# autonomousvision/unimatch

Hardware: AMD Instinct MI355X
Metric: image_pairs_per_sec (higher is better)
Workload: dtype f16x2

## Files before the change

### include/unimatch_hip.h

```cpp
#ifndef UNIMATCH_HIP_H
#define UNIMATCH_HIP_H

#include <stddef.h>
#include <stdint.h>

#ifdef __cplusplus
extern "C" {
#endif

#define UM_VERSION 220

#define UM_MODE_EXACT 0
#define UM_MODE_FAST 1

#define UM_ERR_BAD_ARG (-1)
#define UM_ERR_BAD_GEOMETRY (-2)
#define UM_ERR_WORKSPACE (-3)
#define UM_ERR_UNSUPPORTED (-4)
#define UM_ERR_COLLECTIVE (-5)

int um_version(void);
const char* um_last_error_string(void);

#define UM_RANGE_PLANES 1u
// ... 60 lines not shown
                             const float* gamma, const float* beta, const float* residual, float eps, int wshift, float* out,
                             int streams, int h, int w, int channels, int ldq, int ldkv, long q_plane_stride,
                             long kv_plane_stride, int win_h, int win_w, int shift_h, int shift_w, int kv_rotate, int mode,
                             void* stream);

size_t um_window_attn_ksplit_workspace_bytes(int streams, int h, int w, int win_h, int win_w);
int um_window_attn_plan(int streams, int h, int w, int win_h, int win_w, int* full_tiles, int* split_tiles, int* parts);
int um_window_attn_qproj_merge_fwd(const float* x, const void* wq_planes, const void* k_planes, const void* v_planes,
                                   const void* wm_planes, const float* gamma, const float* beta, const float* residual, float eps,
                                   int wshift, float* out, int streams, int h, int w, int channels, int ldkv,
                                   long kv_plane_stride, int win_h, int win_w, int shift_h, int shift_w, int kv_rotate, int mode,
                                   void* workspace, size_t workspace_bytes, void* stream);

#define UM_EPI_PLANES 0
#define UM_EPI_LN 1
#define UM_EPI_GELU_PLANES 2
size_t um_planes_bytes(long rows, int cols, int mode);
int um_weight_planes(const float* w, void* planes, int n, int k, int wshift, int mode, void* stream);
int um_linear_fwd(const float* a0, const float* a1, const void* a_planes, const void* w_planes,
                  int m, int n, int k, int wshift, int epilogue, void* out,
                  const float* gamma, const float* beta, const float* residual, float eps,
                  int mode, void* stream);

int um_linear_bias_fwd(const float* a0, const void* a_planes, const void* w_planes, const float* bias, int m, int n, int k,
                       int wshift, float out_mul, float bias_mul, void* out_planes, float* out_f32, int mode, void* stream);

int um_ffn_fwd(const float* x, const float* y, const void* w1_planes, const void* w2_planes, int m, int hidden,
               int wshift, const float* gamma, const float* beta, float eps, float* out, int mode, void* stream);
size_t um_ffn_split_workspace_bytes(int m, int hidden);
int um_ffn_ws_fwd(const float* x, const float* y, const void* w1_planes, const void* w2_planes, int m, int hidden,
                  int wshift, const float* gamma, const float* beta, float eps, float* out, int mode, void* workspace,
                  size_t workspace_bytes, void* stream);

int um_kv4_fwd(const float* x, const void* wc_planes, int m, int wshift, void* out_planes, int mode, void* stream);
int um_ffn_kv_fwd(const float* x, const float* y, const void* w1_planes, const void* w2_planes, int m, int hidden, int wshift,
                  const float* gamma, const float* beta, float eps, float* out, const void* wc_planes, void* kv_planes, int mode,
                  void* workspace, size_t workspace_bytes, void* stream);

int um_conv2d_fwd(const void* a_planes, const void* w_planes, const float* bias, float* out, float* stats_out, int batch,
                  int hi, int wi, int cin, int cout, int kh, int kw, int stride, int pad_h, int pad_w, int relu, int wshift,
                  int mode, void* stream);
int um_conv2d_ex(const void* a_planes, int a_ld, int a_coff, long a_rows, const void* w_planes, const float* bias, float* out,
                 int out_ld, int out_coff, void* out_planes, int outp_ld, int outp_coff, long outp_rows, float* stats_out,
                 int batch, int hi, int wi, int cin, int cout, int kh, int kw, int stride, int pad_h, int pad_w, int act,
                 int wshift, int mode, void* stream);
int um_conv2d_gru_fwd(int gate, const void* a_planes, int a_ld, int a_coff, long a_rows, const void* w_planes, const float* bias,
                      float* hidden, const float* z, int z_ld, float* z_out, int z_out_ld, void* out_planes, int outp_ld,
                      int outp_coff, long outp_rows, int batch, int hi, int wi, int cin, int channels, int kh, int kw, int pad_h,
                      int pad_w, int wshift, int mode, void* stream);
int um_conv2d_gru_add_fwd(int gate, const void* a_planes, int a_ld, int a_coff, long a_rows, const void* w_planes, const float* bias,
                          const float* addend, int addend_ld, float* hidden, const float* z, int z_ld, float* z_out, int z_out_ld,
                          void* out_planes, int outp_ld, int outp_coff, long outp_rows, int batch, int hi, int wi, int cin,
                          int channels, int kh, int kw, int pad_h, int pad_w, int wshift, int mode, void* stream);
int um_conv_stats_parts(int hi, int wi, int cout, int kh, int kw, int stride, int pad_h, int pad_w);
size_t um_conv_stats_bytes(int batch, int parts, int channels);

size_t um_stem_planes_bytes(int batch, int h, int w);
size_t um_conv7_planes_bytes(int batch, int h, int w, int stride);
int um_conv7_fwd(const float* image, int channels, int normalize, const float* mean3, const float* std3, void* image_planes,
                 const void* w_planes, const float* bias, float* out, int out_ld, int out_coff, void* out_planes, int outp_ld,
                 int outp_coff, long outp_rows, float* stats_out, int batch, int h, int w, int cout, int stride, int act,
                 int wshift, void* stream);
int um_stem_conv_fwd(const float* image, int normalize, const float* mean3, const float* std3, void* image_planes,
                     const void* w_planes, float* out, float* stats_out, int batch, int h, int w, int cout, int wshift,
                     void* stream);

size_t um_nhwc_norm_workspace_bytes(int batch, int pixels, int channels);
int um_nhwc_instance_norm(const float* x, const float* shortcut, const void* shortcut_planes, void* planes_out, float* f32_out,
                          int batch, int pixels, int channels, float eps, int normalize, int relu, const float* conv_stats,
                          int conv_stats_parts, void* workspace, size_t workspace_bytes, int mode, void* stream);

size_t um_nhwc_norm_sc_workspace_bytes(int batch, int pixels, int channels);
int um_nhwc_instance_norm_sc(const float* x, const float* shortcut, const void* shortcut_planes, void* planes_out, float* f32_out,
                             int batch, int pixels, int channels, float eps, int normalize, int relu, const float* conv_stats,
                             int conv_stats_parts, void* workspace, size_t workspace_bytes, int mode, void* stream,
                             const float* sc_conv_stats, int sc_conv_stats_parts);

int um_nhwc_stats_finalize(const float* conv_stats, int conv_stats_parts, float* stats_out, int batch, int pixels, int channels,
                           float eps, void* stream);
int um_conv2d_norm_supported(int hi, int wi, int cin, int cout, int kh, int kw, int stride, int pad_h, int pad_w, int mode);
int um_conv2d_norm_fwd(const float* x, const float* norm_stats, int norm_relu, const void* w_planes, const float* bias, float* out,
                       float* stats_out, int batch, int hi, int wi, int cin, int cout, int kh, int kw, int stride, int pad_h,
                       int pad_w, int relu, int wshift, int mode, void* stream);

int um_conv2d_entry_supported(int hi, int wi, int cin, int cout, int kh, int kw, int stride, int pad_h, int pad_w, int mode);
int um_conv2d_entry_fwd(const float* u, const float* ustats, const void* s_planes, const void* w_planes, const void* w2_planes,
                        const float* bias2, float* out_t, float* out_d, float* stats_t, float* stats_d, int batch, int hi, int wi,
                        int cin, int cout, int kh, int kw, int stride, int pad_h, int pad_w, int wshift, int mode, void* stream);

int um_nhwc_gate(int mode, const float* src, int src_ld, const float* zr, float* hbuf, void* planes_out, int ld, int coff,
                 long plane_rows, long rows, int channels, void* stream);

int um_nchw_to_nhwc(const float* x, void* planes_out, float* f32_out, int batch, int channels, int pixels, int mode,
                    void* stream);

size_t um_global_corr_workspace_bytes(int batch, int tokens, int channels, int mode);
int um_global_corr_softmax_flow(const float* f0, const float* f1, float* flow,
                                int batch, int h, int w, int channels, int bidir,
                                int mode, void* workspace, size_t workspace_bytes, void* stream);

int um_global_corr_softmax_stereo(const float* f0, const float* f1, float* disp,
                                  int batch, int h, int w, int channels,
                                  int mode, void* workspace, size_t workspace_bytes, void* stream);

int um_prop_global_attn(const float* q, const float* k, const float* value, float* out,
                        int batch, int h, int w, int channels, int value_channels,
                        int mode, void* workspace, size_t workspace_bytes, void* stream);
float um_global_corr_plane_scale(int channels);
int um_prop_global_attn_planes(const void* q_planes, const void* k_planes, const float* value, float* out, int batch, int h,
                               int w, int channels, int value_channels, int mode, void* workspace, size_t workspace_bytes,
                               void* stream);


int um_local_corr_softmax(const float* f0, const float* f1, float* out,
                          int batch, int h, int w, int channels, int radius, int one_d, void* stream);

int um_local_corr_with_flow(const float* f0, const float* f1, const float* flow, float* cost,
                            int batch, int h, int w, int channels, int radius, void* stream);
int um_local_corr_with_flow_dilated(const float* f0, const float* f1, const float* flow, float* cost,
                                    int batch, int h, int w, int channels, int radius, int dilation, void* stream);
int um_local_corr_with_flow_planes(const float* f0, const float* f1, const float* flow, void* planes_out, int ld, long plane_rows,
                                   int batch, int h, int w, int channels, int radius, void* stream);

// ... 102 lines not shown
```

### unimatch_amd/_abi.py

```python
import ctypes
import os

_HERE = os.path.dirname(os.path.abspath(__file__))
LIB_PATH = os.environ.get('UM_LIB') or os.path.join(_HERE, 'libunimatch_hip.so')

MODE_EXACT = 0
MODE_FAST = 1

CENSUS = {'wattn_tile': 0, 'wattn_ksplit': 1, 'ffn_tile': 2, 'ffn_hsplit': 3, 'gsv4': 4, 'gsv3': 5, 'k4_mfma': 6, 'k4_valu': 7,
          'k3_mfma': 8, 'k3_valu': 9, 'conv_patch': 10, 'conv_rows': 11, 'conv_generic': 12, 'wattn_w8': 13, 'conv_patch_norm': 14}

_c_int, _c_size_t, _c_void_p = ctypes.c_int, ctypes.c_size_t, ctypes.c_void_p

SIGNATURES = {
    'um_version': (_c_int, []),
    'um_last_error_string': (ctypes.c_char_p, []),
    'um_range_flags': (_c_int, [ctypes.POINTER(ctypes.c_uint), _c_int]),
    'um_timing_enable': (_c_int, [_c_int]),
    'um_timing_collect': (_c_int, [_c_int, ctypes.POINTER(ctypes.c_double), ctypes.POINTER(_c_int)]),
    'um_window_attn_workspace_bytes': (_c_size_t, [_c_int] * 4),
    'um_window_attn_fwd': (_c_int, [_c_void_p] * 4 + [_c_int] * 9 + [_c_void_p, _c_size_t, _c_void_p]),
    'um_window_attn_planes_fwd': (_c_int, [_c_void_p] * 4 + [_c_int] * 6 + [ctypes.c_long] * 2 + [_c_int] * 6 + [_c_void_p]),
    'um_window_attn_merge_fwd': (_c_int, [_c_void_p] * 7 + [ctypes.c_float, _c_int, _c_void_p] + [_c_int] * 6 + [ctypes.c_long] * 2 +
                                 [_c_int] * 6 + [_c_void_p]),
    'um_window_attn_qproj_merge_fwd': (_c_int, [_c_void_p] * 8 + [ctypes.c_float, _c_int, _c_void_p] + [_c_int] * 5 + [ctypes.c_long] +
                                       [_c_int] * 6 + [_c_void_p, _c_size_t, _c_void_p]),
    'um_window_attn_ksplit_workspace_bytes': (_c_size_t, [_c_int] * 5),
    'um_window_attn_plan': (_c_int, [_c_int] * 5 + [ctypes.POINTER(_c_int)] * 3),
    'um_planes_bytes': (_c_size_t, [ctypes.c_long, _c_int, _c_int]),
    'um_weight_planes': (_c_int, [_c_void_p] * 2 + [_c_int] * 4 + [_c_void_p]),
    'um_linear_fwd': (_c_int, [_c_void_p] * 4 + [_c_int] * 5 + [_c_void_p] * 4 + [ctypes.c_float, _c_int, _c_void_p]),
    'um_linear_bias_fwd': (_c_int, [_c_void_p] * 4 + [_c_int] * 4 + [ctypes.c_float] * 2 + [_c_void_p] * 2 + [_c_int, _c_void_p]),
    'um_ffn_fwd': (_c_int, [_c_void_p] * 4 + [_c_int] * 3 + [_c_void_p] * 2 + [ctypes.c_float, _c_void_p, _c_int, _c_void_p]),
    'um_ffn_ws_fwd': (_c_int, [_c_void_p] * 4 + [_c_int] * 3 + [_c_void_p] * 2 + [ctypes.c_float, _c_void_p, _c_int, _c_void_p, _c_size_t,
                                _c_void_p]),
    'um_ffn_split_workspace_bytes': (_c_size_t, [_c_int] * 2),
    'um_ffn_kv_fwd': (_c_int, [_c_void_p] * 4 + [_c_int] * 3 + [_c_void_p] * 2 + [ctypes.c_float, _c_void_p, _c_void_p, _c_void_p, _c_int, _c_void_p,
                                _c_size_t, _c_void_p]),
    'um_kv4_fwd': (_c_int, [_c_void_p, _c_void_p, _c_int, _c_int, _c_void_p, _c_int, _c_void_p]),
    'um_conv2d_fwd': (_c_int, [_c_void_p] * 5 + [_c_int] * 13 + [_c_void_p]),
    'um_conv2d_ex': (_c_int, [_c_void_p, _c_int, _c_int, ctypes.c_long, _c_void_p, _c_void_p, _c_void_p, _c_int, _c_int, _c_void_p,
                              _c_int, _c_int, ctypes.c_long, _c_void_p] + [_c_int] * 13 + [_c_void_p]),
    'um_nhwc_gate': (_c_int, [_c_int, _c_void_p, _c_int, _c_void_p, _c_void_p, _c_void_p, _c_int, _c_int, ctypes.c_long, ctypes.c_long,
                              _c_int, _c_void_p]),
    'um_local_corr_with_flow_planes': (_c_int, [_c_void_p] * 4 + [_c_int, ctypes.c_long] + [_c_int] * 5 + [_c_void_p]),
    'um_conv2d_gru_fwd': (_c_int, [_c_int, _c_void_p, _c_int, _c_int, ctypes.c_long, _c_void_p, _c_void_p, _c_void_p, _c_void_p, _c_int,
                                   _c_void_p, _c_int, _c_void_p, _c_int, _c_int, ctypes.c_long] + [_c_int] * 11 + [_c_void_p]),
    'um_conv2d_gru_add_fwd': (_c_int, [_c_int, _c_void_p, _c_int, _c_int, ctypes.c_long, _c_void_p, _c_void_p, _c_void_p, _c_int, _c_void_p, _c_void_p,
                                        _c_int, _c_void_p, _c_int, _c_void_p, _c_int, _c_int, ctypes.c_long] + [_c_int] * 11 + [_c_void_p]),
    'um_conv2d_norm_supported': (_c_int, [_c_int] * 10),
    'um_conv2d_norm_fwd': (_c_int, [_c_void_p, _c_void_p, _c_int] + [_c_void_p] * 4 + [_c_int] * 13 + [_c_void_p]),
    'um_conv2d_entry_supported': (_c_int, [_c_int] * 10),
    'um_conv2d_entry_fwd': (_c_int, [_c_void_p] * 10 + [_c_int] * 12 + [_c_void_p]),
    'um_nhwc_norm_sc_workspace_bytes': (_c_size_t, [_c_int] * 3),
    'um_nhwc_instance_norm_sc': (_c_int, [_c_void_p] * 5 + [_c_int] * 3 + [ctypes.c_float, _c_int, _c_int, _c_void_p, _c_int, _c_void_p,
                                          _c_size_t, _c_int, _c_void_p, _c_void_p, _c_int]),
    'um_nhwc_stats_finalize': (_c_int, [_c_void_p, _c_int, _c_void_p] + [_c_int] * 3 + [ctypes.c_float, _c_void_p]),
    'um_conv_stats_bytes': (_c_size_t, [_c_int] * 3),
    'um_conv_stats_parts': (_c_int, [_c_int] * 8),
    'um_stem_planes_bytes': (_c_size_t, [_c_int] * 3),
    'um_conv7_planes_bytes': (_c_size_t, [_c_int] * 4),
    'um_conv7_fwd': (_c_int, [_c_void_p, _c_int, _c_int] + [_c_void_p] * 6 + [_c_int, _c_int, _c_void_p, _c_int, _c_int, ctypes.c_long,
                              _c_void_p] + [_c_int] * 7 + [_c_void_p]),
    'um_stem_conv_fwd': (_c_int, [_c_void_p, _c_int] + [_c_void_p] * 6 + [_c_int] * 5 + [_c_void_p]),
    'um_nhwc_norm_workspace_bytes': (_c_size_t, [_c_int] * 3),
    'um_nhwc_instance_norm': (_c_int, [_c_void_p] * 5 + [_c_int] * 3 + [ctypes.c_float, _c_int, _c_int, _c_void_p, _c_int, _c_void_p,
                                       _c_size_t, _c_int, _c_void_p]),
    'um_nchw_to_nhwc': (_c_int, [_c_void_p] * 3 + [_c_int] * 4 + [_c_void_p]),
    'um_flow_warp': (_c_int, [_c_void_p] * 3 + [_c_int] * 4 + [_c_void_p]),
    'um_fwd_bwd_occlusion': (_c_int, [_c_void_p] * 4 + [_c_int] * 3 + [ctypes.c_float] * 2 + [_c_void_p]),
    'um_flow_to_rgb_workspace_bytes': (_c_size_t, [_c_int] * 3),
    'um_flow_to_rgb': (_c_int, [_c_void_p] * 2 + [_c_int] * 3 + [_c_void_p, _c_size_t, _c_void_p]),
    'um_flow_metrics_workspace_bytes': (_c_size_t, [_c_int] * 3),
    'um_flow_metrics': (_c_int, [_c_void_p] * 5 + [_c_int] * 7 + [_c_void_p, _c_size_t, _c_void_p]),
    'um_disp_metrics_workspace_bytes': (_c_size_t, [_c_int] * 3),
    'um_disp_metrics': (_c_int, [_c_void_p] * 3 + [_c_int] * 7 + [ctypes.c_float, _c_void_p, _c_size_t, _c_void_p]),
    'um_depth_metrics_workspace_bytes': (_c_size_t, [_c_int] * 3),
    'um_depth_metrics': (_c_int, [_c_void_p] * 4 + [_c_int] * 7 + [ctypes.c_float] * 2 + [_c_void_p, _c_size_t, _c_void_p]),
    'um_image_prepare': (_c_int, [_c_void_p, _c_int, _c_void_p] + [_c_int] * 4 + [ctypes.POINTER(ctypes.c_float)] * 2 + [_c_int] * 5 +
                         [_c_void_p]),
    'um_pred_restore': (_c_int, [_c_void_p] * 2 + [_c_int] * 11 + [_c_void_p]),
    'um_convex_upsample': (_c_int, [_c_void_p] * 3 + [_c_int] * 7 + [_c_void_p]),
    'um_flow_upsample2x': (_c_int, [_c_void_p] * 2 + [_c_int] * 4 + [ctypes.c_float, _c_void_p]),
    'um_depth_cam_pack': (_c_int, [_c_void_p] * 3 + [_c_int, ctypes.c_float, _c_int, _c_void_p]),
    'um_rigid_flow': (_c_int, [_c_void_p] * 3 + [_c_int] * 3 + [_c_void_p]),
    'um_instance_norm_fwd': (_c_int, [_c_void_p] * 3 + [ctypes.c_long, _c_int, ctypes.c_float, _c_int, _c_void_p]),
    'um_global_corr_workspace_bytes': (_c_size_t, [_c_int] * 4),
    'um_global_corr_softmax_flow': (_c_int, [_c_void_p] * 3 + [_c_int] * 6 + [_c_void_p, _c_size_t, _c_void_p]),
    'um_global_corr_softmax_stereo': (_c_int, [_c_void_p] * 3 + [_c_int] * 5 + [_c_void_p, _c_size_t, _c_void_p]),
    'um_prop_global_attn': (_c_int, [_c_void_p] * 4 + [_c_int] * 6 + [_c_void_p, _c_size_t, _c_void_p]),
    'um_global_corr_plane_scale': (ctypes.c_float, [_c_int]),
    'um_prop_global_attn_planes': (_c_int, [_c_void_p] * 4 + [_c_int] * 6 + [_c_void_p, _c_size_t, _c_void_p]),
    'um_local_corr_softmax': (_c_int, [_c_void_p] * 3 + [_c_int] * 6 + [_c_void_p]),
    'um_local_corr_with_flow': (_c_int, [_c_void_p] * 4 + [_c_int] * 5 + [_c_void_p]),
    'um_local_corr_with_flow_dilated': (_c_int, [_c_void_p] * 4 + [_c_int] * 6 + [_c_void_p]),
    'um_local_corr_feat_planes_bytes': (ctypes.c_size_t, [_c_int] * 4),
    'um_local_corr_feat_planes': (_c_int, [_c_void_p] * 3 + [_c_int] * 4 + [_c_void_p]),
    'um_local_corr_with_flow_feat_supported': (_c_int, [_c_int] * 4),
    'um_local_corr_softmax_mfma': (_c_int, [_c_void_p] * 3 + [_c_int] * 5 + [_c_void_p, ctypes.c_size_t, _c_void_p]),
    'um_local_corr_with_flow_feat': (_c_int, [_c_void_p] * 6 + [_c_int, ctypes.c_long] + [_c_int] * 6 + [_c_void_p, _c_void_p]),
    'um_prop_local_attn': (_c_int, [_c_void_p] * 4 + [_c_int] * 6 + [_c_void_p]),
    'um_depth_corr_softmax': (_c_int, [_c_void_p] * 5 + [_c_int] * 6 + [_c_void_p]),
    'um_census_enable': (_c_int, [_c_int]),
    'um_census_count': (ctypes.c_long, [_c_int]),
    'um_window_attn_tile_census': (_c_int, [_c_int, ctypes.POINTER(ctypes.c_ulonglong)]),
    'um_probe_mfma_flops': (ctypes.c_double, [_c_int]),
    'um_probe_mfma': (_c_int, [_c_void_p, _c_int, _c_void_p]),
    'um_probe_copy': (_c_int, [_c_void_p, _c_void_p, _c_size_t, _c_void_p]),
    'um_probe_chase': (_c_int, [_c_void_p, _c_void_p, _c_int, _c_void_p]),
    'um_swin_attn_fwd': (_c_int, [_c_void_p] * 4 + [_c_int] * 9 + [_c_void_p, _c_size_t, _c_void_p]),
    'um_attn1d_fwd': (_c_int, [_c_void_p] * 4 + [_c_int] * 7 + [_c_void_p, _c_size_t, _c_void_p]),
    'um_local_corr_softmax_1d': (_c_int, [_c_void_p] * 3 + [_c_int] * 5 + [_c_void_p]),
    **{f'um_workspace_bytes_{op}': (_c_size_t, [_c_int] * 5) for op in (
        'swin_attn_fwd', 'attn1d_fwd', 'global_corr_softmax_flow', 'global_corr_softmax_stereo', 'prop_global_attn',
        'local_corr_softmax', 'local_corr_softmax_1d', 'local_corr_with_flow', 'prop_local_attn', 'depth_corr_softmax',
        'allgather_preds')},
    'um_comm_unique_id': (_c_int, [_c_void_p]),
# ... 100 lines not shown
```

### unimatch_amd/csrc/conv.hip

```cpp
#include <cstdlib>
#include <cstring>
#ifndef UM_CONV_2P
#define UM_CONV_2P 0
#endif
#include "common.h"
#include "planes.h"

struct ConvArgs {
    const unsigned short* ap;
    long a_plane_stride;
    unsigned row_stride;
    unsigned zero_row;
    const unsigned short* wp;
    long w_plane_stride;
    const float* bias;
    float* out;
    unsigned short* outp;
    long outp_plane_stride;
    int out_ld, out_coff, outp_ld, outp_coff;
    int act;
    int gate, gate_c, gate_zld;
    float* gate_h;
    const float* gate_z;
    float* gate_hout;
    int gate_hout_ld;
    float* stats;
    const float* addend;
    int addend_ld;
    int B, Hi, Wi, Cin, Ho, Wo, Cout;
    int KH, KW, stride, pad_h, pad_w;
    int M;
    float out_scale;
    int xcd;
    const float* xf;
    const float* nstats;
    int norm_relu;
};

__device__ __forceinline__ void conv_dma16(const void* base, unsigned byte_off, const unsigned char* lds_dst) {
    const unsigned dst = __builtin_amdgcn_readfirstlane(
        (unsigned)(unsigned long)(const __attribute__((address_space(3))) unsigned char*)lds_dst);
    unsigned keep;
    asm volatile("s_mov_b32 %0, m0\n\ts_mov_b32 m0, %3\n\ts_nop 0\n\tglobal_load_lds_dwordx4 %1, %2\n\ts_mov_b32 m0, %0"
                 : "=&s"(keep)
                 : "v"(byte_off), "s"(base), "s"(dst)
                 : "memory");
}

template <int V>
struct IntC {
    static constexpr int value = V;
};

template <typename T, int NS, int NT, int NT0, int NTP, int WSTRIDE>
__device__ __forceinline__ void conv_epilogue_pass(const ConvArgs& a, f32x16 (&acc)[NT], unsigned char* lds, unsigned char* scratch,
                                                   int bt, int rloc0, int nvalid, int part0, bool dense_parts, int n0, int tid,
                                                   int wave, int lane, int half) {
    const int P = a.Ho * a.Wo;
    constexpr int ROWB = 32 * NTP * 4;
    const int nb = n0 + 32 * NT0;
    unsigned char* stg = lds + wave * WSTRIDE;
    const int tl = lane & 31;
    constexpr int CPR = 8 * NTP;
    constexpr int ITER = 32 * CPR / 64;
    constexpr int BATCH = ITER < 4 ? ITER : 4, NBATCH = ITER / BATCH, NSIDE = NT == 4 ? 2 : 1;
    static_assert(ITER % BATCH == 0, "batches cover the iterations");
    const long rowbase = (long)bt * P + rloc0;
    const int nrows = nvalid;
    const int gate = a.gate;
    float* hbase = gate ? a.gate_h + rowbase * a.gate_c : nullptr;
    const float* zbase = gate == 2 ? a.gate_z + rowbase * a.gate_zld : nullptr;
    const float* abase = a.addend ? a.addend + rowbase * a.addend_ld : nullptr;
    float* hobase = gate == 2 ? a.gate_hout + rowbase * a.gate_hout_ld : nullptr;
    f32x4 ad[NSIDE][BATCH], gz[NSIDE][BATCH], gh[NSIDE][BATCH];
    auto preload = [&](int b, int slot) {
        if (!abase && !gate) return;
#pragma unroll
        for (int j = 0; j < BATCH; ++j) {
            const int idx = (b * BATCH + j) * 64 + lane;
            const int r = idx / CPR, c = idx - r * CPR;
            const int col = nb + 4 * c;
            if (r < nrows && col < a.Cout) {
                if (abase) ad[slot][j] = *reinterpret_cast<const f32x4*>(abase + (unsigned)(r * a.addend_ld + col));
                if (gate == 1 && col >= a.gate_c) gh[slot][j] = *reinterpret_cast<const f32x4*>(hbase + (unsigned)(r * a.gate_c + col - a.gate_c));
                if (gate == 2) {
                    gz[slot][j] = *reinterpret_cast<const f32x4*>(zbase + (unsigned)(r * a.gate_zld + col));
                    gh[slot][j] = *reinterpret_cast<const f32x4*>(hbase + (unsigned)(r * a.gate_c + col));
                }
            }
        }
    };
    preload(0, 0);
    auto to_lds = [&](auto act_tag, auto bias_tag) {
        constexpr int ACT = decltype(act_tag)::value;
        constexpr bool BIAS = decltype(bias_tag)::value != 0;
#pragma unroll
        for (int nt = 0; nt < NTP; ++nt)
#pragma unroll
            for (int g = 0; g < 4; ++g) {
                const int n = nb + 32 * nt + 8 * g + 4 * half;
                f32x4 v;
#pragma unroll
                for (int i = 0; i < 4; ++i) v[i] = acc[NT0 + nt][4 * g + i] * a.out_scale;
                if (BIAS) v = v + *reinterpret_cast<const f32x4*>(a.bias + min(n, a.Cout - 4));
#pragma unroll
                for (int i = 0; i < 4; ++i) {
                    if (ACT == 1) v[i] = fmaxf(v[i], 0.f);
                    else if (ACT == 2) v[i] = 1.0f / (1.0f + __expf(-v[i]));
                    else if (ACT == 3) v[i] = tanhf(v[i]);
                }
                const int c = 8 * nt + 2 * g + half;
                *reinterpret_cast<f32x4*>(stg + tl * ROWB + ((c ^ (tl & 7)) << 4)) = v;
            }
    };
    auto to_lds_b = [&](auto act_tag) {
        if (a.bias) to_lds(act_tag, IntC<1>{});
        else to_lds(act_tag, IntC<0>{});
    };
    switch (a.addend ? 0 : a.act) {
        case 0: to_lds_b(IntC<0>{}); break;
        case 1: to_lds_b(IntC<1>{}); break;
        case 2: to_lds_b(IntC<2>{}); break;
        default: to_lds_b(IntC<3>{}); break;
    }
    __builtin_amdgcn_wave_barrier();
    if (a.stats) {
        constexpr int RG = 64 / CPR >= 8 ? 8 : 64 / CPR >= 4 ? 4 : 2;
        constexpr int RPG = 32 / RG;
        const int nv = nvalid;
        const int c = lane % CPR, rg = lane / CPR;
        const f32x4 k = *reinterpret_cast<const f32x4*>(stg + (c << 4));
        f32x4 s1 = {0.f, 0.f, 0.f, 0.f}, s2 = {0.f, 0.f, 0.f, 0.f};
        if (rg < RG) {
            if (nv == 32) {
#pragma unroll
                for (int j = 0; j < RPG; ++j) {
                    const int r = rg * RPG + j;
                    const f32x4 d = *reinterpret_cast<const f32x4*>(stg + r * ROWB + ((c ^ (r & 7)) << 4)) - k;
                    s1 = s1 + d;
                    s2 = s2 + d * d;
                }
            } else {
#pragma unroll
                for (int j = 0; j < RPG; ++j) {
                    const int r = rg * RPG + j;
                    f32x4 d = *reinterpret_cast<const f32x4*>(stg + r * ROWB + ((c ^ (r & 7)) << 4)) - k;
                    if (r >= nv) d = f32x4{0.f, 0.f, 0.f, 0.f};
                    s1 = s1 + d;
                    s2 = s2 + d * d;
                }
            }
        }
#pragma unroll
        for (int step = CPR * RG / 2; step >= CPR; step >>= 1)
#pragma unroll
            for (int i = 0; i < 4; ++i) {
                s1[i] += __shfl_down(s1[i], step, 64);
                s2[i] += __shfl_down(s2[i], step, 64);
            }
        float* ws = reinterpret_cast<float*>(scratch) + wave * (2 * 32 * NT) + 32 * NT0;
        float* cnt = reinterpret_cast<float*>(scratch) + 8 * (2 * 32 * NT);
        if (lane == 0) cnt[wave] = (float)nv;
        if (lane < CPR) {
            const float inv = nv > 0 ? 1.0f / (float)nv : 0.f;
            *reinterpret_cast<f32x4*>(ws + 4 * c) = k + s1 * inv;
            *reinterpret_cast<f32x4*>(ws + 32 * NT + 4 * c) = s2 - s1 * s1 * inv;
        }
        __syncthreads();
        const int grp = tid >> 8, gt = tid & 255;
        if (gt < 32 * NTP && nb + gt < a.Cout && (cnt[4 * grp] > 0.f || dense_parts)) {
            const float* w0 = reinterpret_cast<const float*>(scratch) + grp * 4 * (2 * 32 * NT) + 32 * NT0;
            float mean = w0[gt], m2 = w0[32 * NT + gt];
// ... 21 lines not shown
        float* obase = a.out ? a.out + rowbase * a.out_ld + a.out_coff : nullptr;
        unsigned short* pbase = a.outp ? a.outp + rowbase * a.outp_ld + a.outp_coff : nullptr;
#pragma unroll
        for (int b = 0; b < NBATCH; ++b) {
            const int slot = NSIDE == 2 ? (b & 1) : 0;
            if ((ADD || GATE != 0) && NSIDE == 2 && b + 1 < NBATCH) preload(b + 1, (b + 1) & 1);
            if ((ADD || GATE != 0) && NSIDE == 1 && b > 0) preload(b, 0);
#pragma unroll
            for (int j = 0; j < BATCH; ++j) {
                const int idx = (b * BATCH + j) * 64 + lane;
                const int r = idx / CPR, c = idx - r * CPR;
                f32x4 d = *reinterpret_cast<const f32x4*>(stg + r * ROWB + ((c ^ (r & 7)) << 4));
                int col = nb + 4 * c;
                if (r < nrows && col < a.Cout) {
                    if (ADD) {
                        d = d + ad[slot][j];
#pragma unroll
                        for (int i = 0; i < 4; ++i) {
                            if (a.act == 1) d[i] = fmaxf(d[i], 0.f);
                            else if (a.act == 2) d[i] = 1.0f / (1.0f + __expf(-d[i]));
                            else if (a.act == 3) d[i] = tanhf(d[i]);
                        }
                    }
                    bool to_out = obase != nullptr, to_planes = pbase != nullptr;
                    if (GATE == 1) {
                        if (col >= a.gate_c) {
                            col -= a.gate_c;
                            d = d * gh[slot][j];
                            to_out = false;
                        } else {
                            to_planes = false;
                        }
                    } else if (GATE == 2) {
#pragma unroll
                        for (int i = 0; i < 4; ++i) d[i] = (1.0f - gz[slot][j][i]) * gh[slot][j][i] + gz[slot][j][i] * d[i];
                        *reinterpret_cast<f32x4*>(hobase + (unsigned)(r * a.gate_hout_ld + col)) = d;
                    }
                    if (to_out) __builtin_nontemporal_store(d, reinterpret_cast<f32x4*>(obase + (unsigned)(r * a.out_ld + col)));
                    if (to_planes) {
                        unsigned short* dst = pbase + (unsigned)(r * a.outp_ld + col);
                        const unsigned h0 = T::pack2(d[0], d[1]), h1 = T::pack2(d[2], d[3]);
                        *reinterpret_cast<u32x2*>(dst) = u32x2{h0, h1};
                        if (NS == 2) {
                            const f32x2 u0 = T::unpack2(h0), u1 = T::unpack2(h1);
                            const u32x2 lo = u32x2{T::pack2(d[0] - u0[0], d[1] - u0[1]), T::pack2(d[2] - u1[0], d[3] - u1[1])};
                            *reinterpret_cast<u32x2*>(dst + a.outp_plane_stride) = lo;
                        }
                    }
                }
            }
        }
    };
    auto store_rows_g = [&](auto gate_tag) {
        if (a.addend) store_rows(gate_tag, IntC<1>{});
        else store_rows(gate_tag, IntC<0>{});
    };
    if (a.gate == 0) store_rows_g(IntC<0>{});
    else if (a.gate == 1) store_rows_g(IntC<1>{});
    else store_rows_g(IntC<2>{});
}

template <typename T, int NS, int NT, int NTE = NT>
__device__ __forceinline__ void conv_epilogue(const ConvArgs& a, f32x16 (&acc)[NT], unsigned char* lds, unsigned char* scratch,
                                              int bt, int rloc0, int nvalid, int part0, bool dense_parts, int n0, int tid, int wave,
                                              int lane, int half) {
    constexpr int NP = NTE < NT ? NTE : NT;
    constexpr int WSTRIDE = 32 * (32 * NP * 4);
    conv_epilogue_pass<T, NS, NT, 0, NP, WSTRIDE>(a, acc, lds, scratch, bt, rloc0, nvalid, part0, dense_parts, n0, tid, wave, lane, half);
    if constexpr (NTE < NT)
        conv_epilogue_pass<T, NS, NT, NTE, NT - NTE, WSTRIDE>(a, acc, lds, scratch, bt, rloc0, nvalid, part0, dense_parts, n0, tid, wave,
                                                              lane, half);
}

struct ConvEntryArgs {
    const float* u;
    const float* ustats;
    const unsigned short* sp;
    long s_plane_stride;
    const unsigned short* wp2;
    long w2_plane_stride;
    const float* bias2;
    float* out2;
    float* stats2;
};

template <int NS, int NT>
struct ConvLds {
    static constexpr int TILE = 128 * 64;
    static constexpr int WTILE = 32 * NT * 64;
    static constexpr int STAGE = NS * (TILE + WTILE);
    static constexpr int EPI = 4 * 32 * (32 * NT * 4);
    static constexpr int RING = (2 * STAGE > EPI) ? 2 * STAGE : EPI;
    static constexpr int TOTAL = RING + 8 * 2 * 32 * NT * 4 + 64;
    static constexpr int ENTRY_CIN = 128;
    static constexpr int ENTRY_TOTAL = TOTAL + 2 * ENTRY_CIN * 4;
};

template <typename T, int NS, int NT, bool ENTRY>
__device__ __forceinline__ void conv_body(const ConvArgs& a, const ConvEntryArgs& e, unsigned char* lds) {
    using L = ConvLds<NS, NT>;
    constexpr int TILE = L::TILE, WTILE = L::WTILE, STAGE = L::STAGE, RING = L::RING;

    const int tid = threadIdx.x, lane = tid & 63;
    const int wave = __builtin_amdgcn_readfirstlane(tid >> 6);
    const int half = lane >> 5;
    const int P = a.Ho * a.Wo, tpi = (P + 127) / 128;
    const int ny = (a.Cout + 32 * NT - 1) / (32 * NT);
    const int wg = a.xcd ? xcd_remap(blockIdx.x, gridDim.x) : blockIdx.x;
    const int tile = wg / ny;
    const int bt = tile / tpi, pl0 = (tile - bt * tpi) * 128;
    const int n0 = (wg - tile * ny) * (32 * NT);
    const int cpt = a.Cin >> 5;
    const int nstage = a.KH * a.KW * cpt;
    const int ktot = a.KH * a.KW * a.Cin;

    const int dcp = lane & 3;
    int py[2], px[2], pbase[2];
    bool pok[2];
#pragma unroll
    for (int i = 0; i < 2; ++i) {
        const int p = pl0 + 32 * wave + 16 * i + (lane >> 2);
        pok[i] = p < P;
        const int rem = pok[i] ? p : 0;
// ... 161 lines not shown
            if (centre) proj_load(pcc, 0);
        }
        if (s + 1 < nstage) {
            stage_async(cc * 32, (s + 1) * 32, nxt);
            if constexpr (ENTRY) entry_load(cc * 32);
            advance();
        }
        const unsigned char* at = cur + 32 * wave * 64;
        const unsigned char* wt = cur + NS * TILE;
        __builtin_amdgcn_s_setprio(1);
#pragma unroll
        for (int ks = 0; ks < 2; ++ks) {
            const i16x8 bh = *reinterpret_cast<const i16x8*>(at + foff[ks]);
            i16x8 bl;
            if (NS == 2) bl = *reinterpret_cast<const i16x8*>(at + TILE + foff[ks]);
#pragma unroll
            for (int nt = 0; nt < NT; ++nt) {
                const i16x8 wh = *reinterpret_cast<const i16x8*>(wt + nt * 32 * 64 + foff[ks]);
                if (NS == 2) {
                    const i16x8 wl = *reinterpret_cast<const i16x8*>(wt + WTILE + nt * 32 * 64 + foff[ks]);
                    if (UM_CONV_2P != 1) acc[nt] = T::mfma(wl, bh, acc[nt]);
                    if (UM_CONV_2P != 2) acc[nt] = T::mfma(wh, bl, acc[nt]);
                }
                acc[nt] = T::mfma(wh, bh, acc[nt]);
            }
            if constexpr (ENTRY) {
                if (centre) {
#pragma unroll
                    for (int nt = 0; nt < NT; ++nt) {
                        if (NS == 2) {
                            if (UM_CONV_2P != 1) acc2[nt] = T::mfma(pwl[nt], bh, acc2[nt]);
                            if (UM_CONV_2P != 2) acc2[nt] = T::mfma(pwh[nt], bl, acc2[nt]);
                        }
                        acc2[nt] = T::mfma(pwh[nt], bh, acc2[nt]);
                    }
                    if (ks == 0) proj_load(pcc, 1);
                }
            }
        }
        __builtin_amdgcn_s_setprio(0);
        if constexpr (ENTRY) {
            if (s + 1 < nstage) entry_store(nxt);
            if (++pcc == cpt) {
                pcc = 0;
                ++ptap;
            }
        }
        asm volatile("s_waitcnt vmcnt(0)" ::: "memory");
        __syncthreads();
    }

    {
        const int rloc0 = pl0 + 32 * wave;
        conv_epilogue<T, NS, NT>(a, acc, lds, lds + RING, bt, rloc0, min(32, max(0, P - rloc0)), bt * ((P + 127) / 128) + pl0 / 128, false,
                                 n0, tid, wave, lane, half);
        if constexpr (ENTRY) {
            ConvArgs a2 = a;
            a2.bias = e.bias2;
            a2.out = e.out2;
            a2.stats = e.stats2;
            __syncthreads();
            conv_epilogue<T, NS, NT>(a2, acc2, lds, lds + RING, bt, rloc0, min(32, max(0, P - rloc0)), bt * ((P + 127) / 128) + pl0 / 128,
                                     false, n0, tid, wave, lane, half);
        }
    }
}

template <typename T, int NS, int NT>
__global__ __launch_bounds__(256, 2) void conv_kernel(ConvArgs a) {
    __shared__ __attribute__((aligned(16))) unsigned char lds[ConvLds<NS, NT>::TOTAL];
    conv_body<T, NS, NT, false>(a, ConvEntryArgs{}, lds);
}

template <typename T, int NS, int NT>
__global__ __launch_bounds__(256, 2) void conv_entry_kernel(ConvArgs a, ConvEntryArgs e) {
    __shared__ __attribute__((aligned(16))) unsigned char lds[ConvLds<NS, NT>::ENTRY_TOTAL];
    conv_body<T, NS, NT, true>(a, e, lds);
}

template <int NS, int NT, int KW, int NSLOT>
struct ConvRowsLds {
    static constexpr int NTE = NT < 2 ? NT : 2;
    static constexpr int ATILE = 288 * 32;
    static constexpr int WTILE = 32 * NT * 32;
    static constexpr int STAGE = NS * (ATILE + KW * WTILE);
    static constexpr int EPI = 8 * 32 * (32 * NTE * 4);
    static constexpr int RING = (NSLOT * STAGE > EPI) ? NSLOT * STAGE : EPI;
    static constexpr int TOTAL = RING + 8 * 2 * 32 * NT * 4 + 64;
};

__device__ __forceinline__ void conv_wait_vm(int n) {
    switch (n) {
        case 0: asm volatile("s_waitcnt vmcnt(0)" ::: "memory"); break;
        case 1: asm volatile("s_waitcnt vmcnt(1)" ::: "memory"); break;
        case 2: asm volatile("s_waitcnt vmcnt(2)" ::: "memory"); break;
        case 3: asm volatile("s_waitcnt vmcnt(3)" ::: "memory"); break;
        case 4: asm volatile("s_waitcnt vmcnt(4)" ::: "memory"); break;
        case 6: asm volatile("s_waitcnt vmcnt(6)" ::: "memory"); break;
        case 8: asm volatile("s_waitcnt vmcnt(8)" ::: "memory"); break;
        case 9: asm volatile("s_waitcnt vmcnt(9)" ::: "memory"); break;
        case 12: asm volatile("s_waitcnt vmcnt(12)" ::: "memory"); break;
        case 16: asm volatile("s_waitcnt vmcnt(16)" ::: "memory"); break;
        case 18: asm volatile("s_waitcnt vmcnt(18)" ::: "memory"); break;
        case 24: asm volatile("s_waitcnt vmcnt(24)" ::: "memory"); break;
        default: asm volatile("s_waitcnt vmcnt(0)" ::: "memory"); break;
    }
}

template <typename T, int NS, int NT, int KW, int NSLOT>
__global__ __launch_bounds__(512, (NSLOT == 2 && NT < 4 ? 2 : 1)) void conv_rows_kernel(ConvArgs a) {
    using L = ConvRowsLds<NS, NT, KW, NSLOT>;
    constexpr int ATILE = L::ATILE, WTILE = L::WTILE, STAGE = L::STAGE, RING = L::RING;
    extern __shared__ __attribute__((aligned(16))) unsigned char lds[];

    const int tid = threadIdx.x, lane = tid & 63;
// ... 471 lines not shown
    static const bool rows_enabled = um_debug_env("UM_CONV_NO_ROWS") == nullptr;
    static const char* patch_env = um_debug_env("UM_CONV_PATCH");
    static const char* patch_nts = patch_env ? patch_env : "234";
    const bool same = stride == 1 && ho == hi && wo == wi && (long)ho * wo >= 256 && rows_enabled;
    const bool rows3 = same && kw == 3 && pad_w == 1, rows5 = same && kw == 5 && pad_w == 2 && nt == 4;
    const long tiled = (long)((ho + 7) / 8 * 8) * ((wo + 31) / 32 * 32);
    if (rows3 && kh == 3 && pad_h == 1 && 4L * ho * wo >= 3 * tiled && strchr(patch_nts, '0' + nt) != nullptr) {
        if (cout <= 32) *nt_out = 1;
        return CONV_PATCH;
    }
    return rows3 || rows5 ? CONV_ROWS : CONV_GENERIC;
}

static constexpr bool kNormOnLoad[5] = {false, false, true, true, true};

extern "C" int um_conv2d_norm_supported(int hi, int wi, int cin, int cout, int kh, int kw, int stride, int pad_h, int pad_w, int mode) {
    if (hi <= 0 || wi <= 0 || cin <= 0 || cin % 32 != 0 || cout <= 0 || cout % 4 != 0 || kh <= 0 || kw <= 0 || stride <= 0 || pad_h < 0 ||
        pad_w < 0 || (mode != 0 && mode != 1))
        return 0;
    const int ho = (hi + 2 * pad_h - kh) / stride + 1, wo = (wi + 2 * pad_w - kw) / stride + 1;
    if (ho <= 0 || wo <= 0) return 0;
    int nt;
    if (conv_pick(hi, wi, ho, wo, cout, kh, kw, stride, pad_h, pad_w, &nt) != CONV_PATCH) return 0;
    return nt >= 2 && nt <= 4 && kNormOnLoad[nt] ? 1 : 0;
}

static constexpr bool kEntryConv[5] = {false, false, false, true, true};

extern "C" int um_conv2d_entry_supported(int hi, int wi, int cin, int cout, int kh, int kw, int stride, int pad_h, int pad_w, int mode) {
    if (hi <= 0 || wi <= 0 || cin <= 0 || cin % 32 != 0 || cin > ConvLds<2, 4>::ENTRY_CIN || cout <= 0 || cout % 4 != 0 ||
        (mode != 0 && mode != 1))
        return 0;
    if (kh != 3 || kw != 3 || stride != 2 || pad_h != 1 || pad_w != 1) return 0;
    const int ho = (hi - 1) / 2 + 1, wo = (wi - 1) / 2 + 1;
    int nt;
    if (conv_pick(hi, wi, ho, wo, cout, 3, 3, 2, 1, 1, &nt) != CONV_GENERIC) return 0;
    return nt >= 3 && nt <= 4 && kEntryConv[nt] ? 1 : 0;
}

extern "C" int um_conv_stats_parts(int hi, int wi, int cout, int kh, int kw, int stride, int pad_h, int pad_w) {
    if (hi <= 0 || wi <= 0 || cout <= 0 || kh <= 0 || kw <= 0 || stride <= 0 || pad_h < 0 || pad_w < 0) return -1;
    const int ho = (hi + 2 * pad_h - kh) / stride + 1, wo = (wi + 2 * pad_w - kw) / stride + 1;
    if (ho <= 0 || wo <= 0) return -1;
    int nt;
    if (conv_pick(hi, wi, ho, wo, cout, kh, kw, stride, pad_h, pad_w, &nt) == CONV_PATCH) return 2 * ((ho + 7) / 8) * ((wo + 31) / 32);
    return (int)(((long)ho * wo + 127) / 128);
}

static int conv2d_impl(const void* a_planes, int a_ld, int a_coff, long a_rows, const void* w_planes, const float* bias,
                       float* out, int out_ld, int out_coff, void* out_planes, int outp_ld, int outp_coff, long outp_rows,
                       float* stats_out, int batch, int hi, int wi, int cin, int cout, int kh, int kw, int stride,
                       int pad_h, int pad_w, int act, int wshift, int mode, void* stream_, int gate, float* gate_h,
                       const float* gate_z, int gate_zld, const float* addend = nullptr, int addend_ld = 0, float* gate_hout = nullptr,
                       int gate_hout_ld = 0, const float* norm_x = nullptr, const float* norm_stats = nullptr, int norm_relu = 0) {
    const bool norm = norm_x != nullptr;
    if (gate_hout && (gate != 2 || gate_hout_ld < cout || gate_hout_ld % 4 != 0 || ((unsigned long)gate_hout & 15) != 0)) {
        um_set_error("um_conv2d: a separate new-state tensor goes with gate 2 only: 16-byte aligned fp32 [M][ld >= channels, ld %% 4 == 0]");
        return -1;
    }
    if (addend && (addend_ld < cout || addend_ld % 4 != 0 || ((unsigned long)addend & 15) != 0 || stats_out)) {
        um_set_error("um_conv2d: the addend must be 16-byte aligned fp32 [M][ld >= cout, ld %% 4 == 0] (and excludes fused statistics)");
        return -1;
    }
    if ((!a_planes && !norm) || !w_planes || (!out && !out_planes) || batch <= 0 || hi <= 0 || wi <= 0 || cin <= 0 || cin % 32 != 0 ||
        cout <= 0 || cout % 4 != 0 || kh <= 0 || kw <= 0 || stride <= 0 || pad_h < 0 || pad_w < 0 || (mode != 0 && mode != 1) ||
        wshift < 0 || wshift > 14 || act < 0 || act > 3) {
        um_set_error("um_conv2d: bad argument (batch=%d hi=%d wi=%d cin=%d cout=%d k=%dx%d stride=%d pad=%d,%d act=%d; cin must "
                     "be a multiple of 32, cout of 4)", batch, hi, wi, cin, cout, kh, kw, stride, pad_h, pad_w, act);
        return -1;
    }
    const int ho = (hi + 2 * pad_h - kh) / stride + 1, wo = (wi + 2 * pad_w - kw) / stride + 1;
    if (ho <= 0 || wo <= 0) {
        um_set_error("um_conv2d: empty output (%d x %d)", ho, wo);
        return -1;
    }
    const long rows_in = (long)batch * hi * wi, m = (long)batch * ho * wo;
    if (a_ld < a_coff + cin || a_ld % 8 != 0 || a_coff % 8 != 0 || a_rows < rows_in + 1 ||
        (out && (out_ld < out_coff + cout || out_ld % 4 != 0 || out_coff % 4 != 0)) ||
        (out_planes && (outp_ld < outp_coff + (gate == 1 ? cout / 2 : cout) || outp_ld % 4 != 0 || outp_coff % 4 != 0 ||
                        outp_rows < m))) {
        um_set_error("um_conv2d: inconsistent leading dimensions / offsets / row counts");
        return -1;
    }
    if (stats_out && !out) {
        um_set_error("um_conv2d: fused statistics need the fp32 output");
        return -1;
    }
    if (bias && ((unsigned long)bias & 15) != 0) {
        um_set_error("um_conv2d: bias must be 16-byte aligned");
        return -1;
    }
    if (a_rows * a_ld * 2 >= (1L << 32) || (long)cout * kh * kw * cin * 2 >= (1L << 32) || m >= (1L << 31)) {
        um_set_error("um_conv2d: operand planes beyond 4 GiB are not addressable by this kernel");
        return -4;
    }
    if (norm) {
        if (!norm_stats || ((unsigned long)norm_x & 15) != 0 || ((unsigned long)norm_stats & 3) != 0) {
            um_set_error("um_conv2d_norm_fwd: the fp32 input must be 16-byte aligned and comes with its statistics [batch][2][cin]");
            return -1;
        }
        if (!um_conv2d_norm_supported(hi, wi, cin, cout, kh, kw, stride, pad_h, pad_w, mode)) {
            um_set_error("um_conv2d_norm_fwd: no on-load kernel for this geometry (hi=%d wi=%d cin=%d cout=%d k=%dx%d stride=%d pad=%d,%d): "
                         "ask um_conv2d_norm_supported() first", hi, wi, cin, cout, kh, kw, stride, pad_h, pad_w);
            return -2;
        }
        if (rows_in * cin * 4 >= (1L << 32) - 1) {
            um_set_error("um_conv2d_norm_fwd: an fp32 input beyond 4 GiB is not addressable by this kernel");
            return -4;
        }
    }
    ConvArgs a;
    a.xf = norm_x;
    a.nstats = norm_stats;
    a.norm_relu = norm_relu;
    a.ap = (const unsigned short*)a_planes + a_coff;
    a.a_plane_stride = a_rows * a_ld;
    a.row_stride = (unsigned)a_ld * 2;
    a.zero_row = (unsigned)(a_rows - 1);
    a.wp = (const unsigned short*)w_planes;
    a.w_plane_stride = (long)cout * kh * kw * cin;
    a.bias = bias;
    a.out = out;
    a.out_ld = out_ld;
    a.out_coff = out_coff;
    a.outp = (unsigned short*)out_planes;
    a.outp_ld = outp_ld;
    a.outp_coff = outp_coff;
    a.outp_plane_stride = outp_rows * outp_ld;
    a.stats = stats_out;
    a.addend = addend;
    a.addend_ld = addend_ld;
    a.B = batch;
    a.Hi = hi;
    a.Wi = wi;
    a.Cin = cin;
    a.Ho = ho;
    a.Wo = wo;
    a.Cout = cout;
    a.KH = kh;
    a.KW = kw;
    a.stride = stride;
    a.pad_h = pad_h;
    a.pad_w = pad_w;
    a.M = (int)m;
    a.act = act;
    a.gate = gate;
    a.gate_c = gate == 1 ? cout / 2 : cout;
    a.gate_h = gate_h;
    a.gate_z = gate_z;
    a.gate_zld = gate_zld;
    a.gate_hout = gate_hout ? gate_hout : gate_h;
    a.gate_hout_ld = gate_hout ? gate_hout_ld : a.gate_c;
    a.out_scale = ldexpf(1.f, -wshift);
    a.xcd = conv_xcd_enabled();
    hipError_t e;
    int nt;
    const ConvKind kind = conv_pick(hi, wi, ho, wo, cout, kh, kw, stride, pad_h, pad_w, &nt);
    hipStream_t st = (hipStream_t)stream_;
    if (norm)
        e = nt == 2 ? launch_conv_patch<2, true>(a, mode, st) : nt == 3 ? launch_conv_patch<3, true>(a, mode, st) : launch_conv_patch<4, true>(a, mode, st);
    else if (kind == CONV_PATCH)
        e = nt == 1 ? launch_conv_patch<1>(a, mode, st) : nt == 2 ? launch_conv_patch<2>(a, mode, st) : nt == 3 ? launch_conv_patch<3>(a, mode, st)
                                                                                                          : launch_conv_patch<4>(a, mode, st);
    else if (kind == CONV_ROWS && kw == 5) e = launch_conv_rows<4, 5, 2>(a, mode, st);
    else if (kind == CONV_ROWS) e = nt == 2 ? launch_conv_rows<2, 3, 2>(a, mode, st) : nt == 3 ? launch_conv_rows<3, 3, 2>(a, mode, st) : launch_conv_rows<4, 3, 2>(a, mode, st);
    else e = nt == 2 ? launch_conv<2>(a, mode, st) : nt == 3 ? launch_conv<3>(a, mode, st) : launch_conv<4>(a, mode, st);
    if (e != hipSuccess) {
        um_set_error("um_conv2d: launch failed: %s", hipGetErrorString(e));
        return (int)e;
    }
    return 0;
}

extern "C" int um_conv2d_ex(const void* a_planes, int a_ld, int a_coff, long a_rows, const void* w_planes, const float* bias,
                            float* out, int out_ld, int out_coff, void* out_planes, int outp_ld, int outp_coff, long outp_rows,
                            float* stats_out, int batch, int hi, int wi, int cin, int cout, int kh, int kw, int stride,
                            int pad_h, int pad_w, int act, int wshift, int mode, void* stream_) {
    return conv2d_impl(a_planes, a_ld, a_coff, a_rows, w_planes, bias, out, out_ld, out_coff, out_planes, outp_ld, outp_coff,
                       outp_rows, stats_out, batch, hi, wi, cin, cout, kh, kw, stride, pad_h, pad_w, act, wshift, mode, stream_, 0,
                       nullptr, nullptr, 0);
}

extern "C" int um_conv2d_gru_fwd(int gate, const void* a_planes, int a_ld, int a_coff, long a_rows, const void* w_planes,
                                 const float* bias, float* hidden, const float* z, int z_ld, float* z_out, int z_out_ld,
                                 void* out_planes, int outp_ld, int outp_coff, long outp_rows, int batch, int hi, int wi, int cin,
                                 int channels, int kh, int kw, int pad_h, int pad_w, int wshift, int mode, void* stream_) {
    if ((gate != 1 && gate != 2) || !hidden || !out_planes || channels <= 0 || channels % 4 != 0 || (gate == 1 && !z_out) ||
        (gate == 2 && !z)) {
        um_set_error("um_conv2d_gru_fwd: bad argument (gate=%d channels=%d)", gate, channels);
        return -1;
    }
    if (gate == 1)
        return conv2d_impl(a_planes, a_ld, a_coff, a_rows, w_planes, bias, z_out, z_out_ld, 0, out_planes, outp_ld, outp_coff,
                           outp_rows, nullptr, batch, hi, wi, cin, 2 * channels, kh, kw, 1, pad_h, pad_w, 2, wshift, mode, stream_,
                           1, hidden, nullptr, 0);
    return conv2d_impl(a_planes, a_ld, a_coff, a_rows, w_planes, bias, nullptr, 0, 0, out_planes, outp_ld, outp_coff, outp_rows,
                       nullptr, batch, hi, wi, cin, channels, kh, kw, 1, pad_h, pad_w, 3, wshift, mode, stream_, 2, hidden, z, z_ld);
}

extern "C" int um_conv2d_gru_add_fwd(int gate, const void* a_planes, int a_ld, int a_coff, long a_rows, const void* w_planes,
                                     const float* bias, const float* addend, int addend_ld, float* hidden, const float* z, int z_ld,
                                     float* z_out, int z_out_ld, void* out_planes, int outp_ld, int outp_coff, long outp_rows,
                                     int batch, int hi, int wi, int cin, int channels, int kh, int kw, int pad_h, int pad_w,
                                     int wshift, int mode, void* stream_) {
    if ((gate != 1 && gate != 2) || !hidden || !out_planes || !addend || channels <= 0 || channels % 4 != 0 || (gate == 1 && !z_out) ||
        (gate == 2 && !z)) {
        um_set_error("um_conv2d_gru_add_fwd: bad argument (gate=%d channels=%d)", gate, channels);
        return -1;
    }
    if (gate == 1)
        return conv2d_impl(a_planes, a_ld, a_coff, a_rows, w_planes, bias, z_out, z_out_ld, 0, out_planes, outp_ld, outp_coff,
                           outp_rows, nullptr, batch, hi, wi, cin, 2 * channels, kh, kw, 1, pad_h, pad_w, 2, wshift, mode, stream_,
                           1, hidden, nullptr, 0, addend, addend_ld);
    return conv2d_impl(a_planes, a_ld, a_coff, a_rows, w_planes, bias, nullptr, 0, 0, out_planes, outp_ld, outp_coff, outp_rows,
                       nullptr, batch, hi, wi, cin, channels, kh, kw, 1, pad_h, pad_w, 3, wshift, mode, stream_, 2, hidden, z, z_ld,
                       addend, addend_ld, z_out, z_out_ld);
}

extern "C" int um_conv2d_fwd(const void* a_planes, const void* w_planes, const float* bias, float* out, float* stats_out,
                             int batch, int hi, int wi, int cin, int cout, int kh, int kw, int stride, int pad_h, int pad_w,
                             int relu, int wshift, int mode, void* stream_) {
    const long rows_in = (long)batch * hi * wi;
    return um_conv2d_ex(a_planes, cin, 0, rows_in + 1, w_planes, bias, out, cout, 0, nullptr, 0, 0, 0, stats_out, batch, hi, wi,
                        cin, cout, kh, kw, stride, pad_h, pad_w, relu ? 1 : 0, wshift, mode, stream_);
}

extern "C" int um_conv2d_norm_fwd(const float* x, const float* norm_stats, int norm_relu, const void* w_planes, const float* bias, float* out,
                                  float* stats_out, int batch, int hi, int wi, int cin, int cout, int kh, int kw, int stride, int pad_h,
                                  int pad_w, int relu, int wshift, int mode, void* stream_) {
    if (!x) {
        um_set_error("um_conv2d_norm_fwd: no input");
        return -1;
    }
    const long rows_in = (long)batch * hi * wi;
    return conv2d_impl(nullptr, cin, 0, rows_in + 1, w_planes, bias, out, cout, 0, nullptr, 0, 0, 0, stats_out, batch, hi, wi, cin, cout, kh,
                       kw, stride, pad_h, pad_w, relu ? 1 : 0, wshift, mode, stream_, 0, nullptr, nullptr, 0, nullptr, 0, nullptr, 0, x,
                       norm_stats, norm_relu ? 1 : 0);
}

extern "C" int um_conv2d_entry_fwd(const float* u, const float* ustats, const void* s_planes, const void* w_planes, const void* w2_planes,
                                   const float* bias2, float* out_t, float* out_d, float* stats_t, float* stats_d, int batch, int hi, int wi,
                                   int cin, int cout, int kh, int kw, int stride, int pad_h, int pad_w, int wshift, int mode, void* stream_) {
    if (!u || !ustats || !s_planes || !w_planes || !w2_planes || !out_t || !out_d || batch <= 0 || wshift < 0 || wshift > 14) {
        um_set_error("um_conv2d_entry_fwd: bad argument (a null input / output, batch=%d, wshift=%d)", batch, wshift);
        return -1;
    }
    if (!um_conv2d_entry_supported(hi, wi, cin, cout, kh, kw, stride, pad_h, pad_w, mode)) {
        um_set_error("um_conv2d_entry_fwd: no entry kernel for this geometry (hi=%d wi=%d cin=%d cout=%d k=%dx%d stride=%d pad=%d,%d mode=%d): "
                     "ask um_conv2d_entry_supported() first", hi, wi, cin, cout, kh, kw, stride, pad_h, pad_w, mode);
        return -2;
    }
    if ((((unsigned long)u | (unsigned long)s_planes | (unsigned long)w_planes | (unsigned long)w2_planes | (unsigned long)bias2 |
          (unsigned long)out_t | (unsigned long)out_d) & 15) != 0 || (((unsigned long)ustats | (unsigned long)stats_t | (unsigned long)stats_d) & 3) != 0) {
        um_set_error("um_conv2d_entry_fwd: inputs, planes, bias and outputs must be 16-byte aligned");
        return -1;
    }
    const int ho = (hi - 1) / 2 + 1, wo = (wi - 1) / 2 + 1;
    const long rows_in = (long)batch * hi * wi, m = (long)batch * ho * wo;
    if (rows_in * cin * 4 >= (1L << 32) - 1 || (long)cout * 9 * cin * 2 >= (1L << 32) || m >= (1L << 31)) {
        um_set_error("um_conv2d_entry_fwd: an input beyond 4 GiB is not addressable by this kernel");
        return -4;
    }
    ConvArgs a;
    memset(&a, 0, sizeof(a));
    a.wp = (const unsigned short*)w_planes;
    a.w_plane_stride = (long)cout * 9 * cin;
    a.out = out_t;
    a.out_ld = cout;
    a.stats = stats_t;
    a.B = batch;
    a.Hi = hi;
    a.Wi = wi;
    a.Cin = cin;
    a.Ho = ho;
    a.Wo = wo;
    a.Cout = cout;
    a.KH = a.KW = 3;
    a.stride = 2;
    a.pad_h = a.pad_w = 1;
    a.M = (int)m;
    a.gate_c = cout;
    a.out_scale = ldexpf(1.f, -wshift);
    a.xcd = conv_xcd_enabled();
    ConvEntryArgs e;
    e.u = u;
    e.ustats = ustats;
    e.sp = (const unsigned short*)s_planes;
    e.s_plane_stride = (rows_in + 1) * cin;
    e.wp2 = (const unsigned short*)w2_planes;
    e.w2_plane_stride = (long)cout * cin;
    e.bias2 = bias2;
    e.out2 = out_d;
    e.stats2 = stats_d;
    int nt;
    conv_pick(hi, wi, ho, wo, cout, 3, 3, 2, 1, 1, &nt);
    hipStream_t st = (hipStream_t)stream_;
    const hipError_t err = nt == 3 ? launch_conv_entry<3>(a, e, mode, st) : launch_conv_entry<4>(a, e, mode, st);
    if (err != hipSuccess) {
        um_set_error("um_conv2d_entry_fwd: launch failed: %s", hipGetErrorString(err));
        return (int)err;
    }
    return 0;
}

template <int CPP>
__global__ __launch_bounds__(256) void pack7_kernel(const float* img, unsigned short* planes, long plane_stride, int B, int C,
                                                    int H, int W, int Hp, int Wp, int normalize, float m0, float m1, float m2,
                                                    float s0, float s1, float s2) {
    const long idx = (long)blockIdx.x * 256 + threadIdx.x;
    const long total = (long)B * Hp * Wp;
    if (idx >= total) return;
    const int xp = (int)(idx % Wp);
    const long t = idx / Wp;
    const int yp = (int)(t % Hp), b = (int)(t / Hp);
    const int y = yp - 3, x = xp - 3;
    float v[CPP];
#pragma unroll
    for (int c = 0; c < CPP; ++c) v[c] = 0.f;
    if ((unsigned)y < (unsigned)H && (unsigned)x < (unsigned)W) {
        const float mean[3] = {m0, m1, m2}, sd[3] = {s0, s1, s2};
#pragma unroll
        for (int c = 0; c < CPP; ++c) {
            if (c < C) {
                float p = img[(((long)b * C + c) * H + y) * W + x];
                if (normalize && c < 3) p = (p / 255.0f - mean[c]) / sd[c];
                v[c] = p;
            }
        }
    }
#pragma unroll
    for (int c = 0; c < CPP; c += 4) {
        const unsigned h0 = Fp16::pack2(v[c], v[c + 1]), h1 = Fp16::pack2(v[c + 2], v[c + 3]);
        *reinterpret_cast<u32x2*>(planes + idx * CPP + c) = u32x2{h0, h1};
        const f32x2 u0 = Fp16::unpack2(h0), u1 = Fp16::unpack2(h1);
        *reinterpret_cast<u32x2*>(planes + plane_stride + idx * CPP + c) =
            u32x2{Fp16::pack2(v[c] - u0[0], v[c + 1] - u0[1]), Fp16::pack2(v[c + 2] - u1[0], v[c + 3] - u1[1])};
    }
}

static int conv7_wp(int w) { return (w + 8 + 1) & ~1; }

extern "C" size_t um_conv7_planes_bytes(int batch, int h, int w, int stride) {
    if (batch <= 0 || h <= 0 || w <= 0 || (stride != 1 && stride != 2)) return 0;
    const long cpp = stride == 2 ? 4 : 8;
    return (size_t)(2 * ((long)batch * (h + 6) * conv7_wp(w) + 8) * cpp * 2);
}

extern "C" int um_conv7_fwd(const float* image, int channels, int normalize, const float* mean3, const float* std3,
                            void* image_planes, const void* w_planes, const float* bias, float* out, int out_ld, int out_coff,
                            void* out_planes, int outp_ld, int outp_coff, long outp_rows, float* stats_out, int batch, int h,
                            int w, int cout, int stride, int act, int wshift, void* stream_) {
    hipStream_t stream = (hipStream_t)stream_;
    const int cpp = stride == 2 ? 4 : 8;
    if (!image || !image_planes || !w_planes || (!out && !out_planes) || batch <= 0 || h < 7 || w < 7 || cout <= 0 || cout % 4 != 0 ||
        wshift < 0 || wshift > 14 || (stride != 1 && stride != 2) || channels <= 0 || channels > (stride == 2 ? 3 : 8) ||
        (normalize && (!mean3 || !std3)) || act < 0 || act > 3) {
        um_set_error("um_conv7_fwd: bad argument (batch=%d channels=%d h=%d w=%d cout=%d stride=%d)", batch, channels, h, w, cout, stride);
        return -1;
    }
    const int hp = h + 6, wp = conv7_wp(w);
    const int ho = (h - 1) / stride + 1, wo = (w - 1) / stride + 1;
    const long rows = (long)batch * hp * wp, m = (long)batch * ho * wo;
    if ((out && (out_ld < out_coff + cout || out_ld % 4 != 0 || out_coff % 4 != 0)) ||
        (out_planes && (outp_ld < outp_coff + cout || outp_ld % 4 != 0 || outp_coff % 4 != 0 || outp_rows < m))) {
        um_set_error("um_conv7_fwd: inconsistent leading dimensions / offsets / row counts");
        return -1;
    }
    if (stats_out && !out) {
        um_set_error("um_conv7_fwd: fused statistics need the fp32 output");
        return -1;
    }
    if (bias && ((unsigned long)bias & 15) != 0) {
        um_set_error("um_conv7_fwd: bias must be 16-byte aligned");
        return -1;
    }
    if ((rows + 8) * cpp * 2 >= (1L << 32) || m >= (1L << 31)) {
        um_set_error("um_conv7_fwd: image batch beyond the 32-bit addressing of this kernel");
        return -4;
    }
    const long plane_stride = (rows + 8) * cpp;
    {
        ScopedKernelTimer timer(UM_K_CONV, stream);
        const float mm[3] = {normalize ? mean3[0] : 0.f, normalize ? mean3[1] : 0.f, normalize ? mean3[2] : 0.f};
        const float ss[3] = {normalize ? std3[0] : 1.f, normalize ? std3[1] : 1.f, normalize ? std3[2] : 1.f};
        const dim3 grid((unsigned)((rows + 255) / 256));
        if (cpp == 4)
            hipLaunchKernelGGL((pack7_kernel<4>), grid, dim3(256), 0, stream, image, (unsigned short*)image_planes, plane_stride,
                               batch, channels, h, w, hp, wp, normalize, mm[0], mm[1], mm[2], ss[0], ss[1], ss[2]);
        else
            hipLaunchKernelGGL((pack7_kernel<8>), grid, dim3(256), 0, stream, image, (unsigned short*)image_planes, plane_stride,
                               batch, channels, h, w, hp, wp, normalize, mm[0], mm[1], mm[2], ss[0], ss[1], ss[2]);
    }
    ConvArgs a;
    a.ap = (const unsigned short*)image_planes;
    a.a_plane_stride = plane_stride;
    a.row_stride = (unsigned)cpp * 2;
    a.zero_row = 0;
    a.wp = (const unsigned short*)w_planes;
    a.w_plane_stride = (long)cout * 7 * 8 * cpp;
    a.bias = bias;
    a.out = out;
    a.out_ld = out_ld;
    a.out_coff = out_coff;
    a.outp = (unsigned short*)out_planes;
    a.outp_ld = outp_ld;
    a.outp_coff = outp_coff;
    a.outp_plane_stride = outp_rows * outp_ld;
    a.stats = stats_out;
    a.addend = nullptr;
    a.addend_ld = 0;
    a.B = batch;
    a.Hi = hp;
    a.Wi = wp;
    a.Cin = 8 * cpp;
    a.Ho = ho;
    a.Wo = wo;
    a.Cout = cout;
    a.KH = 7;
    a.KW = 1;
    a.stride = stride;
    a.pad_h = 0;
    a.pad_w = 0;
    a.M = (int)m;
    a.act = act;
    a.gate = 0;
    a.gate_c = a.gate_zld = 0;
    a.gate_h = nullptr;
    a.gate_z = nullptr;
    a.out_scale = ldexpf(1.f, -wshift);
    a.xcd = conv_xcd_enabled();
    a.xf = a.nstats = nullptr;
    a.norm_relu = 0;
    hipError_t e;
    if (cout % 128 == 0 || cout > 192) e = launch_conv<4>(a, 0, stream);
    else if (cout % 96 == 0) e = launch_conv<3>(a, 0, stream);
    else e = launch_conv<2>(a, 0, stream);
    if (e != hipSuccess) {
        um_set_error("um_conv7_fwd: launch failed: %s", hipGetErrorString(e));
        return (int)e;
    }
    return 0;
}

extern "C" size_t um_stem_planes_bytes(int batch, int h, int w) { return um_conv7_planes_bytes(batch, h, w, 2); }

extern "C" int um_stem_conv_fwd(const float* image, int normalize, const float* mean3, const float* std3, void* image_planes,
                                const void* w_planes, float* out, float* stats_out, int batch, int h, int w, int cout,
                                int wshift, void* stream_) {
    return um_conv7_fwd(image, 3, normalize, mean3, std3, image_planes, w_planes, nullptr, out, cout, 0, nullptr, 0, 0, 0, stats_out,
                        batch, h, w, cout, 2, 0, wshift, stream_);
}
```

### unimatch_amd/csrc/nhwc_ops.hip

```cpp
#include "common.h"
#include "planes.h"

#define NHWC_CHUNK_ROWS 256

__global__ __launch_bounds__(256) void nhwc_stats_kernel(const float* x, float* partial, int P, int C, int nchunk) {
    __shared__ float red[2][256 * 4];
    const int b = blockIdx.y, ch = blockIdx.x;
    const int quads = C >> 2, rl_n = 256 / quads;
    const int q = threadIdx.x % quads, rl = threadIdx.x / quads;
    const int r0 = ch * NHWC_CHUNK_ROWS, r1 = min(P, r0 + NHWC_CHUNK_ROWS);
    const float* xb = x + ((long)b * P) * C + 4 * q;
    f32x4 s1 = {0.f, 0.f, 0.f, 0.f}, s2 = s1;
    if (rl < rl_n) {
        const f32x4 k = *reinterpret_cast<const f32x4*>(xb + (long)r0 * C);
        for (int r = r0 + rl; r < r1; r += rl_n) {
            const f32x4 v = *reinterpret_cast<const f32x4*>(xb + (long)r * C) - k;
            s1 += v;
            s2 += v * v;
        }
    }
#pragma unroll
    for (int i = 0; i < 4; ++i) {
        red[0][threadIdx.x * 4 + i] = s1[i];
        red[1][threadIdx.x * 4 + i] = s2[i];
// ... 166 lines not shown
        *reinterpret_cast<f32x4*>(outf + row * C + c + 4) = f32x4{v[4], v[5], v[6], v[7]};
    }
    if (planes) {
        *reinterpret_cast<u32x4*>(planes + row * C + c) = h;
        if (NS == 2) *reinterpret_cast<u32x4*>(planes + plane_stride + row * C + c) = l;
    }
}

template <typename T, int NS>
__global__ __launch_bounds__(256) void nchw_to_nhwc_kernel(const float* x, unsigned short* planes, float* outf, int P, int C,
                                                           long rows) {
    __shared__ float tile[256 * 65];
    const int b = blockIdx.y, p0 = blockIdx.x * 64;
    const int px = threadIdx.x & 63;
    for (int c = threadIdx.x >> 6; c < C; c += 4) {
        const int p = min(p0 + px, P - 1);
        tile[c * 65 + px] = x[((long)b * C + c) * P + p];
    }
    __syncthreads();
    const int c8n = C >> 3;
    const long plane_stride = (rows + 1) * C;
    for (int it = threadIdx.x; it < 64 * c8n; it += 256) {
        const int pl_px = it / c8n, c = (it - pl_px * c8n) * 8;
        if (p0 + pl_px >= P) continue;
        const long row = (long)b * P + p0 + pl_px;
        float v[8];
#pragma unroll
        for (int i = 0; i < 8; ++i) v[i] = tile[(c + i) * 65 + pl_px];
        if (outf) {
            *reinterpret_cast<f32x4*>(outf + row * C + c) = f32x4{v[0], v[1], v[2], v[3]};
            *reinterpret_cast<f32x4*>(outf + row * C + c + 4) = f32x4{v[4], v[5], v[6], v[7]};
        }
        if (planes) {
            const u32x4 h = {T::pack2(v[0], v[1]), T::pack2(v[2], v[3]), T::pack2(v[4], v[5]), T::pack2(v[6], v[7])};
            *reinterpret_cast<u32x4*>(planes + row * C + c) = h;
            if (NS == 2) {
                u32x4 l;
#pragma unroll
                for (int i = 0; i < 4; ++i) {
                    const f32x2 u = T::unpack2(h[i]);
                    l[i] = T::pack2(v[2 * i] - u[0], v[2 * i + 1] - u[1]);
                }
                *reinterpret_cast<u32x4*>(planes + plane_stride + row * C + c) = l;
            }
        }
    }
    if (planes && blockIdx.x == 0 && b == 0) {
        for (int c = threadIdx.x; c < C; c += 256)
#pragma unroll
            for (int pl = 0; pl < NS; ++pl) planes[pl * plane_stride + rows * C + c] = 0;
    }
}

__global__ __launch_bounds__(256) void nhwc_gate_kernel(int mode, const float* src, int src_ld, const float* zr, float* hbuf,
                                                        unsigned short* planes, long plane_stride, int ld, int coff, long rows,
                                                        int C) {
    const int c4n = (C + 3) >> 2;
    const long idx = (long)blockIdx.x * 256 + threadIdx.x;
    if (idx >= rows * c4n) return;
    const long row = idx / c4n;
    const int c = (int)(idx - row * c4n) * 4;
    float v[4];
#pragma unroll
    for (int i = 0; i < 4; ++i) {
        const int ci = c + i;
        float x = 0.f;
        if (ci < C) {
            if (mode == 0) x = src[row * src_ld + ci];
            else if (mode == 1) x = zr[row * (2 * C) + C + ci] * hbuf[row * C + ci];
            else {
                const float z = zr[row * (2 * C) + ci];
                x = (1.0f - z) * hbuf[row * C + ci] + z * src[row * src_ld + ci];
                hbuf[row * C + ci] = x;
            }
        }
        v[i] = x;
    }
    if (!planes) return;
    const unsigned h0 = Fp16::pack2(v[0], v[1]), h1 = Fp16::pack2(v[2], v[3]);
    const f32x2 u0 = Fp16::unpack2(h0), u1 = Fp16::unpack2(h1);
    const unsigned l0 = Fp16::pack2(v[0] - u0[0], v[1] - u0[1]), l1 = Fp16::pack2(v[2] - u1[0], v[3] - u1[1]);
    unsigned short* d = planes + row * ld + coff + c;
    if (c + 4 <= C) {
        *reinterpret_cast<u32x2*>(d) = u32x2{h0, h1};
        *reinterpret_cast<u32x2*>(d + plane_stride) = u32x2{l0, l1};
    } else {
        const unsigned hh[2] = {h0, h1}, ll[2] = {l0, l1};
        for (int i = 0; c + i < C; ++i) {
            d[i] = (unsigned short)(hh[i >> 1] >> (16 * (i & 1)));
            d[plane_stride + i] = (unsigned short)(ll[i >> 1] >> (16 * (i & 1)));
        }
    }
}

extern void um_set_error(const char* fmt, ...);

extern "C" size_t um_nhwc_norm_workspace_bytes(int batch, int pixels, int channels) {
    if (batch <= 0 || pixels <= 0 || channels <= 0) return 0;
    const long nchunk = (pixels + NHWC_CHUNK_ROWS - 1) / NHWC_CHUNK_ROWS;
    return (size_t)((long)batch * nchunk * 3 * channels + (long)batch * 2 * channels) * sizeof(float);
}

extern "C" size_t um_conv_stats_bytes(int batch, int parts, int channels) {
    if (batch <= 0 || parts <= 0 || channels <= 0) return 0;
    return (size_t)((long)batch * parts * 3 * channels) * sizeof(float);
}
// ... 102 lines not shown
        um_set_error("um_nhwc_stats_finalize: launch failed: %s", hipGetErrorString(e));
        return (int)e;
    }
    return 0;
}

extern "C" int um_nchw_to_nhwc(const float* x, void* planes_out, float* f32_out, int batch, int channels, int pixels, int mode,
                               void* stream_) {
    hipStream_t stream = (hipStream_t)stream_;
    if (!x || (!planes_out && !f32_out) || batch <= 0 || pixels <= 0 || channels <= 0 || channels % 8 != 0 || channels > 256 ||
        (mode != 0 && mode != 1)) {
        um_set_error("um_nchw_to_nhwc: bad argument (batch=%d channels=%d pixels=%d: channels must be a multiple of 8, <= 256)",
                     batch, channels, pixels);
        return -1;
    }
    const long rows = (long)batch * pixels;
    const dim3 grid((pixels + 63) / 64, batch);
    ScopedKernelTimer timer(UM_K_INSTANCE_NORM, stream);
    if (mode == 0)
        hipLaunchKernelGGL((nchw_to_nhwc_kernel<Fp16, 2>), grid, dim3(256), 0, stream, x, (unsigned short*)planes_out, f32_out,
                           pixels, channels, rows);
    else
        hipLaunchKernelGGL((nchw_to_nhwc_kernel<Bf16, 1>), grid, dim3(256), 0, stream, x, (unsigned short*)planes_out, f32_out,
                           pixels, channels, rows);
    const hipError_t e = hipGetLastError();
    if (e != hipSuccess) {
        um_set_error("um_nchw_to_nhwc: launch failed: %s", hipGetErrorString(e));
        return (int)e;
    }
    return 0;
}

extern "C" int um_nhwc_gate(int mode, const float* src, int src_ld, const float* zr, float* hbuf, void* planes_out, int ld, int coff,
                            long plane_rows, long rows, int channels, void* stream_) {
    hipStream_t stream = (hipStream_t)stream_;
    const bool ok = rows > 0 && channels > 0 && mode >= 0 && mode <= 2 && (mode == 1 || src) && (mode == 0 || (zr && hbuf)) &&
                    (mode == 2 || planes_out) &&
                    (!planes_out || (ld >= coff + channels && plane_rows >= rows && (channels % 4 != 0 || coff % 4 == 0)));
    if (!ok) {
        um_set_error("um_nhwc_gate: bad argument (mode=%d rows=%ld channels=%d ld=%d coff=%d)", mode, rows, channels, ld, coff);
        return -1;
    }
    const long total = rows * ((channels + 3) / 4);
    ScopedKernelTimer timer(UM_K_INSTANCE_NORM, stream);
    hipLaunchKernelGGL(nhwc_gate_kernel, dim3((unsigned)((total + 255) / 256)), dim3(256), 0, stream, mode, src, src_ld, zr, hbuf,
                       (unsigned short*)planes_out, plane_rows * ld, ld, coff, rows, channels);
    const hipError_t e = hipGetLastError();
    if (e != hipSuccess) {
        um_set_error("um_nhwc_gate: launch failed: %s", hipGetErrorString(e));
        return (int)e;
    }
    return 0;
}
```

### unimatch_amd/encoder.py

```python

import collections

import torch
import torch.nn as nn
import torch.nn.functional as F


def _conv3(cin, cout, stride=1):
    return nn.Conv2d(cin, cout, 3, stride=stride, padding=1, bias=False)


_Deferred = collections.namedtuple('_Deferred', 'u stats shortcut_planes')


class _Residual(nn.Module):

    def __init__(self, cin, cout, stride):
        super().__init__()
        self.conv1, self.conv2 = _conv3(cin, cout, stride), _conv3(cout, cout)
        self.norm1, self.norm2 = nn.InstanceNorm2d(cout), nn.InstanceNorm2d(cout)
        self.downsample = None
        if stride != 1 or cin != cout:
            self.norm3 = nn.InstanceNorm2d(cout)
            self.downsample = nn.Sequential(nn.Conv2d(cin, cout, 1, stride=stride), self.norm3)
# ... 45 lines not shown
                op, of = ops.nhwc_norm(u, b, ho * wo, relu=True, shortcut=d, shortcut_stats=dstats, want_planes=True, want_f32=want_f32,
                                       conv_stats=ustats)
                return op, of, b, ho, wo, cout
            _, sc = ops.nhwc_norm(d, b, ho * wo, relu=False, want_planes=False, want_f32=True, conv_stats=dstats)
        op, of = ops.nhwc_norm(u, b, ho * wo, relu=True, shortcut=sc, shortcut_planes=scp, want_planes=True, want_f32=want_f32,
                               conv_stats=ustats)
        return op, of, b, ho, wo, cout


class _SharedStridedConv(nn.Module):

    def __init__(self, channels, num_branch):
        super().__init__()
        self.num_branch = num_branch
        self.weight = nn.Parameter(torch.empty(channels, channels, 3, 3))
        nn.init.kaiming_uniform_(self.weight, nonlinearity='relu')

    def forward(self, x):
        return [F.conv2d(x, self.weight, None, stride=2 ** i, padding=1) for i in range(self.num_branch)]

    def forward_nhwc(self, act, ops):
        planes, _, b, h, w, c = act
        outs = []
        for i in range(self.num_branch):
            o, ho, wo = ops.conv2d_nhwc((planes, b, h, w, c), self.weight, None, 2 ** i, (1, 1))
            outs.append(o.view(b, ho, wo, -1).permute(0, 3, 1, 2))
        return outs


class CNNEncoder(nn.Module):

    def __init__(self, output_dim=128, num_output_scales=1):
        super().__init__()
        self.num_branch = num_output_scales
        d0, d1, d2 = 64, 96, 128
        self.conv1 = nn.Conv2d(3, d0, 7, stride=2, padding=3, bias=False)
        self.norm1 = nn.InstanceNorm2d(d0)
        self.layer1 = nn.Sequential(_Residual(d0, d0, 1), _Residual(d0, d0, 1))
        self.layer2 = nn.Sequential(_Residual(d0, d1, 2), _Residual(d1, d1, 1))
        self.layer3 = nn.Sequential(_Residual(d1, d2, 2 if num_output_scales == 1 else 1), _Residual(d2, d2, 1))
        self.conv2 = nn.Conv2d(d2, output_dim, 1)
        if num_output_scales > 1:
            if num_output_scales > 4:
                raise ValueError('at most 4 output scales')
            self.trident_conv = _SharedStridedConv(output_dim, num_output_scales)
        for m in self.modules():
            if isinstance(m, nn.Conv2d):
                nn.init.kaiming_normal_(m.weight, mode='fan_out', nonlinearity='relu')

    @staticmethod
    def takes_raw_images(ops, x):
        return ops is not None and getattr(ops, 'fused_conv', False) and x.is_cuda

    def forward(self, x, ops=None, input_norm=None):
        if self.takes_raw_images(ops, x):
            return self._forward_nhwc(x, ops, input_norm)
        assert input_norm is None
        if ops is not None and getattr(ops, 'fused_tail', False) and x.is_cuda:
            x = ops.instance_norm(self.conv1(x), relu=True)
            for layer in (self.layer1, self.layer2, self.layer3):
                for block in layer:
                    x = block(x, ops)
            x = self.conv2(x)
        else:
            x = F.relu(self.norm1(self.conv1(x)))
            x = self.conv2(self.layer3(self.layer2(self.layer1(x))))
        return self.trident_conv(x) if self.num_branch > 1 else [x]


    shortcut_f32 = False

    @staticmethod
    def _out_geometry(blk, act):
        _, _, _, h, w, _ = act
        s = blk.conv1.stride[0]
        return (h - 1) // s + 1, (w - 1) // s + 1, blk.conv1.out_channels

    def _forward_nhwc(self, x, ops, input_norm=None):
        b = x.shape[0]
        y, h, w = ops.stem_conv(x.contiguous(), self.conv1.weight, input_norm, stats=True)
        c = y.shape[1]
        keep_f32 = self.shortcut_f32
        planes, f32 = ops.nhwc_norm(y, b, h * w, relu=True, want_planes=True, want_f32=keep_f32, conv_stats=ops.last_conv_stats)
        act = (planes, f32, b, h, w, c)
        blocks = [blk for layer in (self.layer1, self.layer2, self.layer3) for blk in layer]
        for i, blk in enumerate(blocks):
            nxt = blocks[i + 1] if i + 1 < len(blocks) else None
            defer = nxt is not None and blk.downsample is None and nxt.entry_fusable(ops, *self._out_geometry(blk, act))
            act = blk.forward_nhwc(act, ops, want_f32=keep_f32 and nxt is not None and nxt.downsample is None, defer=defer)
        planes, _, b, h, w, c = act
        out, _, _ = ops.conv2d_nhwc((planes, b, h, w, c), self.conv2.weight, self.conv2.bias, 1, (0, 0))
        if self.num_branch == 1:
            return [out.view(b, h, w, -1).permute(0, 3, 1, 2)]
        tp, _ = ops.nhwc_norm(out, b, h * w, normalize=False, relu=False, want_planes=True)
        return self.trident_conv.forward_nhwc((tp, None, b, h, w, out.shape[1]), ops)
```

### unimatch_amd/model.py

```python
import math
import weakref

import torch
import torch.nn as nn
import torch.nn.functional as F

from .encoder import CNNEncoder
from .refine import BasicUpdateBlock, convex_upsample
from .refine_nhwc import NhwcUpdateBlock
from .dist import shard_batch, shard_bounds
from .streams import PartRunner, forward_parts

_IMAGENET_MEAN = (0.485, 0.456, 0.406)
_IMAGENET_STD = (0.229, 0.224, 0.225)


def attention_windows(attn_type, is_self, splits, h, w, with_shift):
    if attn_type == 'swin':
        kind = 'win2d'
    elif attn_type == 'self_swin2d_cross_1d':
        kind = 'win2d' if is_self else 'row'
    elif attn_type == 'self_swin2d_cross_swin1d':
        kind = 'win2d' if is_self else 'winrow'
    else:
# ... 290 lines not shown

    @property
    def ops(self):
        if self._ops is None:
            from .ops import HipOps
            self._ops = HipOps(self._precision)
        return self._ops

    def _position(self, h, w, splits, device):
        assert splits <= 1 or (h % splits == 0 and w % splits == 0), \
            f'feature map {h}x{w} is not divisible by attn_splits={splits}'
        key = (h, w, splits, str(device))
        if key not in self._pos_cache:
            if splits > 1:
                tab = sine_position_tokens(h // splits, w // splits, splits, splits, self.feature_channels)
            else:
                tab = sine_position_tokens(h, w, 1, 1, self.feature_channels)
            self._pos_cache[key] = tab.to(device)
        return self._pos_cache[key]

    def _constants(self, device):
        key = ('imagenet', str(device))
        if key not in self._pos_cache:
            self._pos_cache[key] = (torch.tensor(_IMAGENET_MEAN).view(1, 3, 1, 1).to(device),
                                    torch.tensor(_IMAGENET_STD).view(1, 3, 1, 1).to(device))
        return self._pos_cache[key]

    def _depth_candidates(self, lo, hi, n, device):
        key = ('cand', float(lo), float(hi), int(n), str(device))
        if key not in self._pos_cache:
            self._pos_cache[key] = torch.linspace(lo, hi, n).float().to(device).contiguous()
        return self._pos_cache[key]

    def _convex(self, flow2, mask, is_depth=False):
        ops = self.ops
        if hasattr(ops, 'convex_upsample') and flow2.is_cuda and self.upsample_factor in (4, 8):
            return ops.convex_upsample(flow2, mask, self.upsample_factor, is_depth)
        return convex_upsample(flow2, mask, self.upsample_factor, is_depth=is_depth)

    check_range = True

    def check_operand_range(self, sync=True):
        from . import _abi
        if sync and torch.cuda.is_available():
            torch.cuda.synchronize()
        _abi.check_operand_range()

    def _upsample_mask(self, flow2, f0_map):
        ops = self.ops
        if getattr(ops, 'fused_conv', False) and flow2.is_cuda and self.upsample_factor in (4, 8):
            b, v, h, w = flow2.shape
            rows = b * h * w
            feat = f0_map.permute(0, 2, 3, 1).reshape(rows, -1)
            planes, cin = ops.nhwc_planes_from([flow2.permute(0, 2, 3, 1).reshape(rows, v), feat])
            c1, c2 = self.upsampler[0], self.upsampler[2]
            hid, _, _ = ops.conv2d_nhwc((planes, b, h, w, cin), ops.conv_weight_padded(c1.weight, cin), c1.bias, 1, (1, 1),
                                        relu=True)
            hp, hc = ops.nhwc_planes_from([hid])
            mask, _, _ = ops.conv2d_nhwc((hp, b, h, w, hc), c2.weight, c2.bias, 1, (0, 0))
            return mask, True
        return self.upsampler(torch.cat([flow2, f0_map], 1)), False

    def _upsample(self, flow2, f0_map, is_depth=False):
        mask, nhwc = self._upsample_mask(flow2, f0_map)
        if nhwc:
            return self.ops.convex_upsample(flow2, mask, self.upsample_factor, is_depth, mask_nhwc=True)
        return self._convex(flow2, mask, is_depth=is_depth)

    launch_parts = None

    def forward(self, img0, img1, attn_type=None, attn_splits_list=None, corr_radius_list=None,
                prop_radius_list=None, num_reg_refine=1, pred_bidir_flow=False, task='flow', intrinsics=None,
                pose=None, min_depth=1. / 0.5, max_depth=1. / 10, num_depth_candidates=64,
                depth_from_argmax=False, pred_bidir_depth=False, **kwargs):
        return self._forward_batch(img0, img1, self.launch_parts, attn_type, attn_splits_list, corr_radius_list, prop_radius_list,
                                   num_reg_refine, pred_bidir_flow, task, intrinsics, pose, min_depth, max_depth, num_depth_candidates,
                                   depth_from_argmax, pred_bidir_depth)

    _PREDICT_DEFAULTS = {'flow': (8, 'sintel', 'flow'), 'stereo': (32, 'sintel', 'disparity'), 'depth': (16, 'kitti', 'depth')}

    def predict(self, img0, img1, *, inference_size=None, padding_factor=None, pad_mode=None, transpose='auto', normalize=None,
                **forward_kw):
        from .prepost import InferenceGeometry, geometry_for, image_size
        task = forward_kw.get('task', 'flow')
        if task not in self._PREDICT_DEFAULTS:
            raise ValueError(f'task must be one of {sorted(self._PREDICT_DEFAULTS)}, got {task!r}')
        factor, mode, kind = self._PREDICT_DEFAULTS[task]
        shape = image_size(img0)
        if image_size(img1) != shape or img1.dtype != img0.dtype:
            raise ValueError(f'img0 {tuple(img0.shape)} {img0.dtype} and img1 {tuple(img1.shape)} {img1.dtype} differ')
        if isinstance(transpose, str):
            transpose = InferenceGeometry._resolve_transpose(shape, transpose) and task == 'flow'
        geom = geometry_for(shape, inference_size, padding_factor or factor, pad_mode or mode, transpose)
        if normalize is None:
            normalize = img0.dtype == torch.uint8 and task != 'flow'
        a0, a1 = geom.prepare(img0, img1, normalize=normalize)
        out = dict(self(a0, a1, **forward_kw))
        preds = list(out['flow_preds'])
        preds[-1] = geom.restore(preds[-1], kind)
        out['flow_preds'] = preds
        return out

    def _forward_batch(self, img0, img1, parts, attn_type=None, attn_splits_list=None, corr_radius_list=None,
                       prop_radius_list=None, num_reg_refine=1, pred_bidir_flow=False, task='flow', intrinsics=None,
                       pose=None, min_depth=1. / 0.5, max_depth=1. / 10, num_depth_candidates=64,
                       depth_from_argmax=False, pred_bidir_depth=False, **kwargs):
        if self.training:
            raise RuntimeError('this module implements inference only: call .eval() '
                               '(training-mode auxiliary outputs of the reference are out of scope)')
        kw = dict(attn_type=attn_type, attn_splits_list=attn_splits_list, corr_radius_list=corr_radius_list,
                  prop_radius_list=prop_radius_list, num_reg_refine=num_reg_refine, pred_bidir_flow=pred_bidir_flow, task=task,
                  intrinsics=intrinsics, pose=pose, min_depth=min_depth, max_depth=max_depth,
                  num_depth_candidates=num_depth_candidates, depth_from_argmax=depth_from_argmax, pred_bidir_depth=pred_bidir_depth)
        batch = img0.shape[0]
        parts = self._plan_parts(parts, task, attn_type, batch, img0.shape[-2], img0.shape[-1], img0.is_cuda)
        if parts <= 1:
            return self._forward_one(img0, img1, **kw)

        def prepare(r):
            pk = dict(kw, intrinsics=shard_batch(intrinsics, r, parts), pose=shard_batch(pose, r, parts))
            return shard_batch(img0, r, parts), shard_batch(img1, r, parts), pk

        def compute(r, ins):
            a0, a1, pk = ins
            return self._forward_one(a0, a1, **pk)['flow_preds']

        bidir = 2 if (pred_bidir_flow or pred_bidir_depth) else 1
        return self._runner.run_parts(self, parts, batch, bidir, img0.shape, img0.device, kw, prepare, compute)

    def _plan_parts(self, parts, task, attn_type, batch, height, width, is_cuda):
        if parts is None:
            parts = 1
            if is_cuda and self.debug_taps is None:
                parts = forward_parts(task, attn_type, self.num_scales, self.reg_refine, batch, height, width)
        return min(int(parts), batch)

    def _carry_state(self, frames):
        ops = self._ops
        params = tuple((id(p), p.data_ptr(), p._version) for p in self.parameters())
        return ((weakref.ref(self), None if ops is None else weakref.ref(ops)),
                (str(frames.device), tuple(frames.shape[1:]), getattr(ops, 'cache_generation', None), params))

    def _carry_valid(self, carry, frames):
        refs, key = carry['state']
        now_refs, now_key = self._carry_state(frames)
        return (refs[0]() is self and (refs[1] is None) == (now_refs[1] is None) and (refs[1] is None or refs[1]() is self._ops)
                and key == now_key)

    def forward_sequence(self, frames, attn_type=None, attn_splits_list=None, corr_radius_list=None, prop_radius_list=None,
                         num_reg_refine=1, pred_bidir_flow=False, consistency_check=False, colorize=False, pairs_per_launch=8,
                         carry=None, task='flow'):
        if self.training:
            raise RuntimeError('this module implements inference only: call .eval()')
        if task != 'flow':
            raise NotImplementedError('forward_sequence is optical flow only')
        if consistency_check and not pred_bidir_flow:
            raise AssertionError('consistency_check needs pred_bidir_flow=True (as the reference asserts)')
        if frames.dim() != 4 or frames.shape[1] != 3:
            raise ValueError(f'frames: expected [T, 3, H, W], got {tuple(frames.shape)}')
        if int(pairs_per_launch) < 1:
            raise ValueError('pairs_per_launch must be >= 1')
        if carry is not None and tuple(carry['frame'].shape[1:]) != tuple(frames.shape[1:]):
            raise ValueError(f'carry holds a {tuple(carry["frame"].shape[2:])} frame, frames are {tuple(frames.shape[2:])}')
        pairs = frames.shape[0] - (0 if carry is not None else 1)
        if pairs < 1:
            raise ValueError('no frame pair: give at least two frames, or one with a carry')
        kw = dict(attn_type=attn_type if attn_type is not None else '', attn_splits_list=attn_splits_list,
                  corr_radius_list=corr_radius_list, prop_radius_list=prop_radius_list, num_reg_refine=num_reg_refine,
                  pred_bidir_flow=pred_bidir_flow, task='flow')
        assert len(attn_splits_list) == len(corr_radius_list) == len(prop_radius_list) == self.num_scales
        import contextlib
        from . import video
        dev = frames.device
        ops = self.ops
        if self.check_weights:
            self._check_weight_print()
        if frames.is_cuda and self.check_range and getattr(ops, 'mode', 1) == 0:
            from . import _abi
            _abi.check_operand_range('an earlier forward of this process: ')
        guard = torch.cuda.device(dev) if frames.is_cuda else contextlib.nullcontext()
        step = int(pairs_per_launch)
# ... 16 lines not shown
                prev = [f[f.shape[0] - 1:] for f in feats]
                fwd = pred[:nb]
                out['flow'].append(fwd)
                if pred_bidir_flow:
                    bwd = pred[nb:]
                    out['flow_bwd'].append(bwd)
                    if consistency_check:
                        occ_f, occ_b = video.forward_backward_consistency_check(fwd, bwd)
                        out['occ_fwd'].append(occ_f)
                        out['occ_bwd'].append(occ_b)
                if colorize:
                    out['flow_rgb'].append(video.flow_to_image(fwd))
                    if pred_bidir_flow:
                        out['flow_bwd_rgb'].append(video.flow_to_image(bwd))
            last = frames[frames.shape[0] - 1:]
            result = {k: v[0] if len(v) == 1 else torch.cat(v, 0) for k, v in out.items() if v}
            result['carry'] = {'features': [p.clone() for p in prev], 'frame': last.clone(), 'state': self._carry_state(frames)}
        return result

    def _match_pairs(self, chunk, nb, kw):
        def frames_of(pieces, a, b):
            out, base = [], 0
            for t in pieces:
                lo, hi = max(a, base), min(b, base + t.shape[0])
                if lo < hi:
                    out.append(t[lo - base:hi - base])
                base += t.shape[0]
            return out

        def stream(lo, hi):
            return [torch.cat(frames_of(pieces, lo, hi) + frames_of(pieces, lo + 1, hi + 1), 0) for pieces in chunk]

        ref = chunk[-1][-1]
        h8, w8 = ref.shape[-2:]
        parts = self._plan_parts(self.launch_parts, 'flow', kw['attn_type'], nb, self.upsample_factor * h8, self.upsample_factor * w8,
                                 ref.is_cuda)
        if parts <= 1:
            return self._match(stream(0, nb), nb, **kw)['flow_preds'][0]

        def prepare(r):
            lo, hi = shard_bounds(nb, r, parts)
            return stream(lo, hi), hi - lo

        def compute(r, ins):
            return self._match(ins[0], ins[1], **kw)['flow_preds']

        bidir = 2 if kw['pred_bidir_flow'] else 1
        return self._runner.run_parts(self, parts, nb, bidir, (nb,) + tuple(ref.shape[1:]), ref.device, kw, prepare,
                                      compute)['flow_preds'][0]

    def _forward_one(self, img0, img1, attn_type=None, attn_splits_list=None, corr_radius_list=None,
                     prop_radius_list=None, num_reg_refine=1, pred_bidir_flow=False, task='flow', intrinsics=None,
                     pose=None, min_depth=1. / 0.5, max_depth=1. / 10, num_depth_candidates=64,
                     depth_from_argmax=False, pred_bidir_depth=False):
        if pred_bidir_flow:
            assert task == 'flow'
        if task == 'depth':
            assert self.num_scales == 1
            assert len(attn_splits_list) == len(prop_radius_list) == self.num_scales == 1
        else:
            assert len(attn_splits_list) == len(corr_radius_list) == len(prop_radius_list) == self.num_scales
        ops = self.ops
        if self.check_weights:
            self._check_weight_print()
        attn_type = attn_type if attn_type is not None else ''
        dev = img0.device
        if img0.is_cuda and self.check_range and getattr(ops, 'mode', 1) == 0:
            from . import _abi
            _abi.check_operand_range('an earlier forward of this process: ')

        import contextlib
        guard = torch.cuda.device(dev) if img0.is_cuda else contextlib.nullcontext()
        if img1.device != dev:
            raise ValueError(f'img0 is on {dev} and img1 on {img1.device}')
        with guard, torch.no_grad():
            feats = self._encode((img0, img1), task)
            return self._match(feats, img0.shape[0], attn_type=attn_type, attn_splits_list=attn_splits_list,
                               corr_radius_list=corr_radius_list, prop_radius_list=prop_radius_list, num_reg_refine=num_reg_refine,
                               pred_bidir_flow=pred_bidir_flow, task=task, intrinsics=intrinsics, pose=pose, min_depth=min_depth,
                               max_depth=max_depth, num_depth_candidates=num_depth_candidates, depth_from_argmax=depth_from_argmax,
                               pred_bidir_depth=pred_bidir_depth)

    def _encode(self, images, task='flow'):
        ops = self.ops
        input_norm = None
        if task == 'flow':
            if self.backbone.takes_raw_images(ops, images[0]):
                input_norm = (_IMAGENET_MEAN, _IMAGENET_STD)
            else:
                mean, std = self._constants(images[0].device)
                images = tuple((im / 255. - mean) / std for im in images)
        stack = images[0] if len(images) == 1 else torch.cat(images, 0)
        return self.backbone(stack, ops, input_norm)[::-1]

    def _match(self, feats, nb, attn_type='', attn_splits_list=None, corr_radius_list=None, prop_radius_list=None, num_reg_refine=1,
               pred_bidir_flow=False, task='flow', intrinsics=None, pose=None, min_depth=1. / 0.5, max_depth=1. / 10,
               num_depth_candidates=64, depth_from_argmax=False, pred_bidir_depth=False):
        ops = self.ops
        dev = feats[0].device
        flow, pred = None, None
        for s in range(self.num_scales):
            m0, m1 = feats[s][:nb], feats[s][nb:]
            both = None
            if pred_bidir_flow and s > 0:
                m0, m1 = torch.cat([m0, m1], 0), torch.cat([m1, m0], 0)
                ori0, ori1 = _to_tokens(m0), _to_tokens(m1)
            else:
                both = _to_tokens(feats[s])
                ori0, ori1 = both[:nb], both[nb:]
            h, w = m0.shape[-2:]
            up = self.upsample_factor * 2 ** (self.num_scales - 1 - s)
            if task == 'depth':
                k_cur = intrinsics.clone()
                k_cur[:, :2] = k_cur[:, :2] / up
            if s > 0:
                if hasattr(ops, 'flow_upsample2x') and flow.is_cuda:
                    flow = ops.flow_upsample2x(flow, 2.0)
                else:
                    flow = F.interpolate(flow, scale_factor=2, mode='bilinear', align_corners=True) * 2
            tok1 = ori1
            if flow is not None:
                assert task != 'depth'
                disp = torch.cat([-flow, torch.zeros_like(flow)], 1) if task == 'stereo' else flow
                if hasattr(ops, 'flow_warp') and ori1.is_cuda:
                    tok1 = ops.flow_warp(ori1, disp.contiguous(), h, w)
                else:
                    tok1 = _to_tokens(_warp(m1, disp))
            splits, prop_r = attn_splits_list[s], prop_radius_list[s]
            pos = self._position(h, w, splits, dev)
            if self.debug_taps is not None:
                self.debug_taps[f'backbone0_s{s}'], self.debug_taps[f'backbone1_s{s}'] = m0, m1
            if tok1 is ori1 and both is not None:
                tok0, tok1 = self.transformer(ops, None, None, h, w, attn_type, splits, stream=both + pos)
            else:
                tok0, tok1 = self.transformer(ops, ori0 + pos, tok1 + pos, h, w, attn_type, splits)
            if self.debug_taps is not None:
                self.debug_taps[f'f0_s{s}'], self.debug_taps[f'f1_s{s}'] = _to_map(tok0, h, w), _to_map(tok1, h, w)

            if task == 'depth':
                cand = self._depth_candidates(min_depth, max_depth, num_depth_candidates, dev)
                f0c, f1c = tok0, tok1
                if pred_bidir_depth:
                    f0c, f1c = torch.cat([tok0, tok1], 0), torch.cat([tok1, tok0], 0)
                if hasattr(ops, 'depth_cam') and tok0.is_cuda:
                    cam = ops.depth_cam(intrinsics, pose, float(up), pred_bidir_depth)
                else:
                    kc, pc = k_cur, pose
                    if pred_bidir_depth:
                        kc = k_cur.repeat(2, 1, 1)
                        pc = torch.cat([pose, torch.inverse(pose)], 0)
                    cam = torch.cat([torch.inverse(kc).flatten(1), pc[:, :3, :3].flatten(1), pc[:, :3, 3],
                                     kc.flatten(1)], 1).float().contiguous()
                flow_pred = ops.depth_corr_softmax(f0c, f1c, h, w, cam, cand.contiguous(), depth_from_argmax)
            else:
                radius = corr_radius_list[s]
                if radius == -1:
                    if task == 'flow':
                        flow_pred = ops.global_corr_softmax_flow(tok0, tok1, h, w, pred_bidir_flow)
                    elif task == 'stereo':
                        flow_pred = ops.global_corr_softmax_stereo(tok0, tok1, h, w)
                    else:
                        raise NotImplementedError
                else:
                    if task not in ('flow', 'stereo'):
                        raise NotImplementedError
                    flow_pred = ops.local_corr_softmax(tok0, tok1, h, w, radius, one_d=(task == 'stereo'))
            flow = flow_pred if flow is None else flow + flow_pred
            if task == 'stereo':
                flow = flow.clamp(min=0)
            if self.debug_taps is not None:
                self.debug_taps[f'flow_match_s{s}'] = flow

            if (pred_bidir_flow or pred_bidir_depth) and s == 0:
                tok0 = torch.cat([tok0, tok1], 0)
            flow = self.feature_flow_attn(ops, tok0, flow.contiguous(), h, w,
                                          local_window_attn=prop_r > 0, local_window_radius=prop_r)
            if self.debug_taps is not None:
                self.debug_taps[f'flow_prop_s{s}'] = flow
            if s < self.num_scales - 1:
                continue

            f0_map = _to_map(tok0, h, w)
            if not self.reg_refine:
                if task == 'stereo':
                    pad = torch.cat([-flow, torch.zeros_like(flow)], 1)
                    pred = -self._upsample(pad, f0_map)[:, :1]
                elif task == 'depth':
                    pad = torch.cat([flow, torch.zeros_like(flow)], 1)
                    pred = self._upsample(pad, f0_map, is_depth=True).clamp(min=min_depth, max=max_depth)[:, :1]
                else:
                    pred = self._upsample(flow, f0_map)
                continue
            assert num_reg_refine > 0
            pose_r = pose
            nhwc = None
            if getattr(ops, 'fused_conv', False) and tok0.is_cuda:
                nhwc = NhwcUpdateBlock(ops, self.refine, self.refine_proj)
                nhwc.begin(tok0, tok0.shape[0], h, w, iterations=num_reg_refine)
            else:
                proj = self.refine_proj(f0_map)
                net0, inp = torch.tanh(proj[:, :128]), torch.relu(proj[:, 128:])
            for it in range(num_reg_refine):
                if task == 'stereo':
                    disp = torch.cat([-flow, torch.zeros_like(flow)], 1)
                elif task == 'depth':
                    if pred_bidir_depth and it == 0:
                        ori0, ori1 = torch.cat([ori0, ori1], 0), torch.cat([ori1, ori0], 0)
                    if hasattr(ops, 'rigid_flow') and flow.is_cuda:
                        disp = ops.rigid_flow(flow, cam)
                    else:
                        if pred_bidir_depth and it == 0:
                            k_cur = k_cur.repeat(2, 1, 1)
                            pose_r = torch.cat([pose, torch.inverse(pose)], 0)
                        disp = _rigid_flow(1. / flow.squeeze(1), k_cur, pose_r)
                else:
                    disp = flow
                if nhwc is not None:
                    up_mask, delta = nhwc.iterate(ori0, ori1, disp.contiguous(), flow, it == num_reg_refine - 1)
                else:
                    corr = ops.local_corr_with_flow(ori0, ori1, disp.contiguous(), h, w, 4)
                    _, up_mask, delta = self.refine(net0, inp, corr, flow)
                if task == 'depth':
                    flow = (flow - delta).clamp(min=min_depth, max=max_depth)
                else:
                    flow = flow + delta
                if task == 'stereo':
                    flow = flow.clamp(min=0)
                if self.debug_taps is not None:
                    self.debug_taps[f'flow_it{it}'] = flow
                if it == num_reg_refine - 1:
                    if task == 'depth':
                        pad = torch.cat([flow, torch.zeros_like(flow)], 1)
                        pred = self._upsample(pad, f0_map, is_depth=True).clamp(
                            min=min_depth, max=max_depth)[:, :1]
                    elif nhwc is not None:
                        pred = ops.convex_upsample(flow, up_mask, self.upsample_factor, False, mask_nhwc=True)
                    else:
                        pred = self._convex(flow, up_mask)
        if task == 'stereo':
            pred = pred.squeeze(1)
        if task == 'depth':
            pred = 1. / pred.squeeze(1)
        return {'flow_preds': [pred]}
```

### unimatch_amd/ops.py

```python
import contextlib
import ctypes
import threading
import weakref
from collections import namedtuple

import torch

from . import _abi

PRECISIONS = {'exact': _abi.MODE_EXACT, 'fast': _abi.MODE_FAST}


class KernelTimer:

    def __init__(self):
        self.records = []

    def summary(self):
        torch.cuda.synchronize()
        out = {}
        for name, s, e, meta in self.records:
            d = out.setdefault(name, {'calls': 0, 'ms': 0.0, 'meta': meta})
            d['calls'] += 1
            d['ms'] += s.elapsed_time(e)
# ... 53 lines not shown
        prev, self._scope.token = self._scope.token, token
        owned = {}
        try:
            yield owned
        finally:
            self._scope.token = prev
            for k in [k for k in self._entries if isinstance(k.owner, tuple) and k.owner[0] is token]:
                owned[k] = self._entries.pop(k)

    @contextlib.contextmanager
    def part_scope(self, lane):
        prev, self._scope.lane = self._scope.lane, lane
        try:
            yield
        finally:
            self._scope.lane = prev

    def workspace_scope(self):
        return self._scope.token, self._scope.lane

    def workspace_entries(self):
        return list(self._entries.items())

    def _workspace(self, kind, geometry, nbytes, device, keep):
        scope = self._scope
        owner = self._stream_handle() if scope.token is None else (scope.token, scope.lane)
        buf = self._entries.get((kind, geometry, device, owner))
        if buf is None:
            if self._capturing():
                return torch.zeros(nbytes, dtype=torch.uint8, device=device)
            group = [k for k in self._entries if (k.kind, k.device, k.owner) == (kind, device, owner)]
            for k in group[:max(0, len(group) + 1 - keep)]:
                del self._entries[k]
            buf = self._entries[WorkspaceKey(kind, geometry, device, owner)] = torch.zeros(nbytes, dtype=torch.uint8, device=device)
        return buf

    def release_cached_planes(self):
        for k in [k for k in self._entries if isinstance(k.kind, tuple)]:
            del self._entries[k]


class HipOps(WorkspaceRegistry):

    fused_tail = True
    fused_ffn = True
    fused_merge = True
    fused_qproj = True
    block_kv = True
    refine_hoist = True
    fused_kv = True
    fused_conv = True
    norm_on_load = True
    fused_entry = True
    CONV_MODE = 0
    WSHIFT = 10

    def __init__(self, precision='exact'):
        if precision not in PRECISIONS:
            raise ValueError(f'precision must be one of {sorted(PRECISIONS)}')
        self.lib = _abi.load()
        if not torch.cuda.is_available():
            raise _abi.HipExtensionError('no GPU visible: the UniMatch hot path only runs on the HIP extension')
        self.precision = precision
        self.mode = PRECISIONS[precision]
        self.timer = None
        self.nplanes = 2 if precision == 'exact' else 1
        self._wcache = {}
        self.cache_generation = 0
        WorkspaceRegistry.__init__(self)

    def _ws(self, nbytes, device):
        return torch.empty(max(int(nbytes), 256), dtype=torch.uint8, device=device)

    def _launch(self, name, fn, meta=None):
        if self.timer is None:
            return fn()
        s, e = torch.cuda.Event(enable_timing=True), torch.cuda.Event(enable_timing=True)
        s.record()
        r = fn()
        e.record()
        self.timer.records.append((name, s, e, meta))
        return r

    def window_attention(self, q, k, v, h, w, win_h, win_w, shift_h=0, shift_w=0):
        s, l, c = q.shape
        _check_tokens('q', q, tokens=h * w)
        _check_tokens('k', k, s, l)
        _check_tokens('v', v, s, l)
        out = torch.empty_like(q)
        nbytes = self.lib.um_window_attn_workspace_bytes(s, l, c, self.mode)
        ws = self._ws(nbytes, q.device)
        n = win_h * win_w
        meta = {'flops': 4.0 * s * l * n * c, 'bytes': 4.0 * 4 * s * l * c}
        code = self._launch('window_attn', lambda: self.lib.um_window_attn_fwd(
            _ptr(q), _ptr(k), _ptr(v), _ptr(out), s, h, w, c, win_h, win_w, shift_h, shift_w,
            self.mode, _ptr(ws), ws.numel(), _stream()), meta)
        _abi.check(code, 'um_window_attn_fwd')
        return out

    def _cache_get(self, tag, tensors):
        key = (tag,) + tuple((id(t), t._version, t.data_ptr(), str(t.device), t.dtype) for t in tensors)
        hit = self._wcache.get(key)
        if hit is not None and all(r() is t for r, t in zip(hit[0], tensors)):
            return key, hit[1]
        return key, None

# ... 153 lines not shown
    def window_attention_qproj_merge(self, x, q_weight, k, v, streams, h, w, win_h, win_w, shift_h, shift_w, kv_rotate,
                                     merge_weight, norm, residual=None):
        (kt, krows, kcols, koff), (vt, vrows, vcols, voff) = k[:4], v[:4]
        kps = k[4] if len(k) > 4 else krows * kcols
        if (v[4] if len(v) > 4 else vrows * vcols) != kps:
            raise ValueError('k and v must share their plane stride')
        self._check_rows('x', x, 128)
        if (krows, kcols) != (vrows, vcols) or x.shape[0] != streams * h * w or krows != x.shape[0]:
            raise ValueError('inconsistent plane shapes')
        wqp, nq, kq = self.weight_planes((q_weight,))
        wp, n, kk = self.weight_planes((merge_weight,))
        if (n, kk, nq, kq) != (128, 128, 128, 128):
            raise ValueError('window_attention_qproj_merge: the query and merge weights must be [128, 128]')
        if residual is not None:
            self._check_rows('residual', residual, 128)
        out = torch.empty((streams, h * w, 128), dtype=torch.float32, device=x.device)
        meta = {'flops': 4.0 * streams * h * w * win_h * win_w * 128}
        ks = self._split_workspace('attn_ksplit', (streams, h, w, win_h, win_w), x.device)
        code = self._launch('window_attn', lambda: self.lib.um_window_attn_qproj_merge_fwd(
            _ptr(x), _ptr(wqp), _ptr(kt) + 2 * koff, _ptr(vt) + 2 * voff, _ptr(wp), _ptr(norm.weight), _ptr(norm.bias),
            _ptr(residual) if residual is not None else None, float(norm.eps), self.WSHIFT, _ptr(out), streams, h, w, 128,
            kcols, kps, win_h, win_w, shift_h, shift_w, kv_rotate, self.mode,
            _ptr(ks) if ks is not None else None, ks.numel() if ks is not None else 0, _stream()), meta)
        _abi.check(code, 'um_window_attn_qproj_merge_fwd')
        return out

    def kv4_weight_planes(self, weights):
        key, hit = self._cache_get('kv4', weights)
        if hit is not None:
            return hit
        if len(weights) != 4 or any(tuple(w.shape) != (128, 128) for w in weights):
            raise ValueError('kv4_weight_planes: expected four [128, 128] weights (k_self, v_self, k_cross, v_cross)')
        wc = pack_kv4_weights(weights)
        self._check_weight_range(wc, self.WSHIFT if self.mode == 0 else 0, 'Linear weight')
        planes = torch.empty(self.lib.um_planes_bytes(256, 256, self.mode), dtype=torch.uint8, device=wc.device)
        _abi.check(self.lib.um_weight_planes(_ptr(wc), _ptr(planes), 256, 256, self.WSHIFT, self.mode, _stream()), 'um_weight_planes')
        return self._cache_put(key, weights, planes)

    @staticmethod
    def kv4_slices(kv, m):
        part = lambda j: (kv, m, 128, j * m * 128, 4 * m * 128)
        return (part(0), part(1)), (part(2), part(3))

    def kv4_planes(self, x, weights):
        self._check_rows('x', x, 128)
        wc = self.kv4_weight_planes(weights)
        m = x.shape[0]
        out = torch.empty(self.lib.um_planes_bytes(4 * m, 128, self.mode), dtype=torch.uint8, device=x.device)
        code = self._launch('linear', lambda: self.lib.um_kv4_fwd(_ptr(x), _ptr(wc), m, self.WSHIFT, _ptr(out), self.mode, _stream()),
                            {'flops': 2.0 * m * 512 * 128})
        _abi.check(code, 'um_kv4_fwd')
        return out

    def convex_upsample(self, flow, mask, factor, is_depth=False, mask_nhwc=False):
        b, v, h, w = flow.shape
        want = (b * h * w, 9 * factor * factor) if mask_nhwc else (b, 9 * factor * factor, h, w)
        if not (flow.is_cuda and flow.dtype == torch.float32 and mask.dtype == torch.float32 and tuple(mask.shape) == want):
            raise ValueError(f'convex_upsample: bad shapes flow {tuple(flow.shape)} mask {tuple(mask.shape)}')
        flow, mask = flow.contiguous(), mask.contiguous()
        up = torch.empty((b, v, factor * h, factor * w), dtype=torch.float32, device=flow.device)
        code = self._launch('convex_upsample', lambda: self.lib.um_convex_upsample(
            _ptr(flow), _ptr(mask), _ptr(up), b, v, h, w, factor, int(bool(is_depth)), int(bool(mask_nhwc)), _stream()))
        _abi.check(code, 'um_convex_upsample')
        return up

    def flow_warp(self, tokens, flow, h, w):
        b, l, c = tokens.shape
        if not (tokens.is_cuda and tokens.dtype == torch.float32 and tokens.is_contiguous() and l == h * w
                and tuple(flow.shape) == (b, 2, h, w) and flow.dtype == torch.float32):
            raise ValueError(f'flow_warp: bad shapes tokens {tuple(tokens.shape)} flow {tuple(flow.shape)}')
        flow = flow.contiguous()
        out = torch.empty_like(tokens)
        code = self._launch('convex_upsample', lambda: self.lib.um_flow_warp(
            _ptr(tokens), _ptr(flow), _ptr(out), b, h, w, c, _stream()))
        _abi.check(code, 'um_flow_warp')
        return out

    def fwd_bwd_occlusion(self, fwd, bwd, alpha=0.01, beta=0.5):
        if not (fwd.is_cuda and fwd.dtype == torch.float32 and fwd.dim() == 4 and fwd.shape[1] == 2
                and bwd.shape == fwd.shape and bwd.dtype == torch.float32 and bwd.device == fwd.device):
            raise ValueError(f'fwd_bwd_occlusion: expected two CUDA float32 [B, 2, H, W] flows of one shape, got '
                             f'{tuple(fwd.shape)} {fwd.dtype} and {tuple(bwd.shape)} {bwd.dtype}')
        fwd, bwd = fwd.contiguous(), bwd.contiguous()
        b, _, h, w = fwd.shape
        occ_f = torch.empty((b, h, w), dtype=torch.float32, device=fwd.device)
        occ_b = torch.empty_like(occ_f)
        code = self._launch('fwd_bwd_occlusion', lambda: self.lib.um_fwd_bwd_occlusion(
            _ptr(fwd), _ptr(bwd), _ptr(occ_f), _ptr(occ_b), b, h, w, float(alpha), float(beta), _stream()))
        _abi.check(code, 'um_fwd_bwd_occlusion')
        return occ_f, occ_b

    def flow_to_rgb(self, flow):
        if not (flow.is_cuda and flow.dtype == torch.float32 and flow.dim() == 4 and flow.shape[1] == 2):
            raise ValueError(f'flow_to_rgb: expected a CUDA float32 [B, 2, H, W] flow, got {tuple(flow.shape)} {flow.dtype}')
        flow = flow.contiguous()
        b, _, h, w = flow.shape
        rgb = torch.empty((b, h, w, 3), dtype=torch.uint8, device=flow.device)
        ws = self._ws(self.lib.um_flow_to_rgb_workspace_bytes(b, h, w), flow.device)
        code = self._launch('flow_to_rgb', lambda: self.lib.um_flow_to_rgb(
            _ptr(flow), _ptr(rgb), b, h, w, _ptr(ws), ws.numel(), _stream()))
        _abi.check(code, 'um_flow_to_rgb')
        return rgb

    @staticmethod
    def _check_sizing(name, mode, size, crop):
        if mode not in ('pad', 'resize'):
            raise ValueError(f"{name}: mode must be 'pad' or 'resize', got {mode!r}")
        (hp, wp), (top, left) = (int(s) for s in size), (int(c) for c in crop)
        if hp < 1 or wp < 1:
            raise ValueError(f'{name}: the inference size {hp}x{wp} is empty')
        return (1 if mode == 'resize' else 0), hp, wp, top, left

    def image_prepare(self, images, size, mode='pad', crop=(0, 0), transpose=False, mean=None, std=None):
# ... 93 lines not shown
        if not (flow.is_cuda and flow.dtype == torch.float32 and flow.dim() == 4):
            raise ValueError('flow_upsample2x: expected a CUDA float32 [B, V, h, w] tensor')
        flow = flow.contiguous()
        b, v, h, w = flow.shape
        out = torch.empty((b, v, 2 * h, 2 * w), dtype=torch.float32, device=flow.device)
        _abi.check(self.lib.um_flow_upsample2x(_ptr(flow), _ptr(out), b, v, h, w, float(mult), _stream()), 'um_flow_upsample2x')
        return out

    def depth_cam(self, intrinsics, pose, stride_div, bidir=False):
        b = intrinsics.shape[0]
        if not (tuple(intrinsics.shape) == (b, 3, 3) and tuple(pose.shape) == (b, 4, 4) and intrinsics.is_cuda and pose.is_cuda):
            raise ValueError('depth_cam: expected CUDA intrinsics [B,3,3] and pose [B,4,4]')
        k, p = intrinsics.float().contiguous(), pose.float().contiguous()
        cam = torch.empty((2 * b if bidir else b, 30), dtype=torch.float32, device=k.device)
        _abi.check(self.lib.um_depth_cam_pack(_ptr(k), _ptr(p), _ptr(cam), b, float(stride_div), int(bool(bidir)), _stream()),
                   'um_depth_cam_pack')
        return cam

    def rigid_flow(self, inv_depth, cam):
        b, _, h, w = inv_depth.shape
        if not (inv_depth.is_cuda and inv_depth.dtype == torch.float32 and tuple(cam.shape) == (b, 30)):
            raise ValueError('rigid_flow: expected CUDA float32 inv_depth [B,1,h,w] and cam [B,30]')
        inv_depth = inv_depth.contiguous()
        out = torch.empty((b, 2, h, w), dtype=torch.float32, device=inv_depth.device)
        _abi.check(self.lib.um_rigid_flow(_ptr(inv_depth), _ptr(cam), _ptr(out), b, h, w, _stream()), 'um_rigid_flow')
        return out

    def instance_norm(self, x, relu=True, shortcut=None, eps=1e-5):
        if not (x.is_cuda and x.dtype == torch.float32 and x.dim() == 4 and x.is_contiguous()):
            raise ValueError('instance_norm: expected a contiguous CUDA float32 NCHW tensor')
        if shortcut is not None and not (shortcut.shape == x.shape and shortcut.is_contiguous()
                                         and shortcut.dtype == torch.float32):
            raise ValueError('instance_norm: shortcut must match x')
        n, c, h, w = x.shape
        y = torch.empty_like(x)
        code = self._launch('instance_norm', lambda: self.lib.um_instance_norm_fwd(
            _ptr(x), _ptr(shortcut) if shortcut is not None else None, _ptr(y), n * c, h * w, float(eps),
            int(bool(relu)), _stream()))
        _abi.check(code, 'um_instance_norm_fwd')
        return y

    def conv_weight_planes(self, weight):
        key, hit = self._cache_get('conv', (weight,))
        if hit is not None:
            return hit
        cout, cin, kh, kw = weight.shape
        w2 = weight.detach().float().permute(0, 2, 3, 1).reshape(cout, kh * kw * cin).contiguous()
        planes = torch.empty(self.lib.um_planes_bytes(cout, kh * kw * cin, self.CONV_MODE), dtype=torch.uint8, device=w2.device)
        self._check_weight_range(w2, self.WSHIFT, 'convolution weight')
        _abi.check(self.lib.um_weight_planes(_ptr(w2), _ptr(planes), cout, kh * kw * cin, self.WSHIFT, self.CONV_MODE, _stream()),
                   'um_weight_planes')
        return self._cache_put(key, (weight,), (planes, cout, cin, kh, kw))

    def conv2d_nhwc(self, act, weight, bias=None, stride=1, padding=(1, 1), relu=False, stats=False):
        planes, b, h, w, cin = act
        wp, cout, wcin, kh, kw = self.conv_weight_planes(weight)
        if wcin != cin:
            raise ValueError(f'conv2d_nhwc: weight expects {wcin} input channels, activation has {cin}')
        ph, pw = (padding, padding) if isinstance(padding, int) else padding
        ho, wo = (h + 2 * ph - kh) // stride + 1, (w + 2 * pw - kw) // stride + 1
        out = torch.empty((b * ho * wo, cout), dtype=torch.float32, device=planes.device)
        self.last_conv_stats = None
        if stats:
            parts = self.lib.um_conv_stats_parts(h, w, cout, kh, kw, stride, ph, pw)
            self.last_conv_stats = (torch.empty(self.lib.um_conv_stats_bytes(b, parts, cout) // 4, dtype=torch.float32,
                                                device=planes.device), parts)
        st = self.last_conv_stats[0] if self.last_conv_stats is not None else None
        meta = {'flops': 2.0 * b * ho * wo * cout * kh * kw * cin}
        code = self._launch('conv', lambda: self.lib.um_conv2d_fwd(
            _ptr(planes), _ptr(wp), _ptr(bias) if bias is not None else None, _ptr(out), _ptr(st) if st is not None else None,
            b, h, w, cin, cout, kh, kw,
            stride, ph, pw, int(bool(relu)), self.WSHIFT, self.CONV_MODE, _stream()), meta)
        _abi.check(code, 'um_conv2d_fwd')
        return out, ho, wo

    def conv2d_norm_supported(self, h, w, cin, weight, stride=1, padding=(1, 1)):
        cout, wcin, kh, kw = weight.shape
        ph, pw = (padding, padding) if isinstance(padding, int) else padding
        return wcin == cin and bool(self.lib.um_conv2d_norm_supported(h, w, cin, cout, kh, kw, stride, ph, pw, self.CONV_MODE))

    def conv2d_nhwc_normed(self, x, conv_stats, geom, weight, bias=None, norm_relu=True, relu=False, stats=False, eps=1e-5):
        b, h, w, cin = geom
        self._check_rows('x', x, cin)
        if x.shape[0] != b * h * w:
            raise ValueError('conv2d_nhwc_normed: x must have b * h * w rows')
        wp, cout, wcin, kh, kw = self.conv_weight_planes(weight)
        if wcin != cin:
            raise ValueError(f'conv2d_nhwc_normed: weight expects {wcin} input channels, activation has {cin}')
        nstats = torch.empty((b, 2, cin), dtype=torch.float32, device=x.device)
        _abi.check(self._launch('instance_norm', lambda: self.lib.um_nhwc_stats_finalize(
            _ptr(conv_stats[0]), conv_stats[1], _ptr(nstats), b, h * w, cin, float(eps), _stream())), 'um_nhwc_stats_finalize')
        out = torch.empty((b * h * w, cout), dtype=torch.float32, device=x.device)
        self.last_conv_stats = None
        if stats:
            parts = self.lib.um_conv_stats_parts(h, w, cout, kh, kw, 1, 1, 1)
            self.last_conv_stats = (torch.empty(self.lib.um_conv_stats_bytes(b, parts, cout) // 4, dtype=torch.float32,
                                                device=x.device), parts)
        st = self.last_conv_stats[0] if self.last_conv_stats is not None else None
        meta = {'flops': 2.0 * b * h * w * cout * kh * kw * cin}
        code = self._launch('conv', lambda: self.lib.um_conv2d_norm_fwd(
            _ptr(x), _ptr(nstats), int(bool(norm_relu)), _ptr(wp), _ptr(bias) if bias is not None else None, _ptr(out),
            _ptr(st) if st is not None else None, b, h, w, cin, cout, kh, kw, 1, 1, 1, int(bool(relu)), self.WSHIFT, self.CONV_MODE,
            _stream()), meta)
        _abi.check(code, 'um_conv2d_norm_fwd')
        return out, h, w

    def conv2d_entry_supported(self, h, w, cin, weight, proj_weight, stride=2, padding=(1, 1)):
        cout, wcin, kh, kw = weight.shape
        ph, pw = (padding, padding) if isinstance(padding, int) else padding
        return (wcin == cin and tuple(proj_weight.shape) == (cout, cin, 1, 1) and
                bool(self.lib.um_conv2d_entry_supported(h, w, cin, cout, kh, kw, stride, ph, pw, self.CONV_MODE)))

    def conv2d_entry(self, u, conv_stats, shortcut_planes, geom, weight, proj_weight, proj_bias, eps=1e-5):
        b, h, w, cin = geom
        self._check_rows('u', u, cin)
        if u.shape[0] != b * h * w:
            raise ValueError('conv2d_entry: u must have b * h * w rows')
        if shortcut_planes.numel() != self.lib.um_planes_bytes(b * h * w + 1, cin, self.CONV_MODE):
            raise ValueError('conv2d_entry: shortcut_planes must be operand planes of [b * h * w + 1, cin]')
        wp, cout, wcin, kh, kw = self.conv_weight_planes(weight)
        wp2, cout2, wcin2, kh2, kw2 = self.conv_weight_planes(proj_weight)
        if wcin != cin or (cout2, wcin2, kh2, kw2) != (cout, cin, 1, 1):
            raise ValueError('conv2d_entry: the weights do not fit the activation / each other')
        nstats = torch.empty((b, 2, cin), dtype=torch.float32, device=u.device)
        _abi.check(self._launch('instance_norm', lambda: self.lib.um_nhwc_stats_finalize(
            _ptr(conv_stats[0]), conv_stats[1], _ptr(nstats), b, h * w, cin, float(eps), _stream())), 'um_nhwc_stats_finalize')
        ho, wo = (h - 1) // 2 + 1, (w - 1) // 2 + 1
        t = torch.empty((b * ho * wo, cout), dtype=torch.float32, device=u.device)
        d = torch.empty_like(t)
        parts = self.lib.um_conv_stats_parts(h, w, cout, 3, 3, 2, 1, 1)
        nst = self.lib.um_conv_stats_bytes(b, parts, cout) // 4
        st_t = torch.empty(nst, dtype=torch.float32, device=u.device)
        st_d = torch.empty(nst, dtype=torch.float32, device=u.device)
        meta = {'flops': 2.0 * b * ho * wo * cout * 10 * cin}
        code = self._launch('conv', lambda: self.lib.um_conv2d_entry_fwd(
            _ptr(u), _ptr(nstats), _ptr(shortcut_planes), _ptr(wp), _ptr(wp2), _ptr(proj_bias) if proj_bias is not None else None, _ptr(t), _ptr(d), _ptr(st_t), _ptr(st_d),
            b, h, w, cin, cout, 3, 3, 2, 1, 1, self.WSHIFT, self.CONV_MODE, _stream()), meta)
        _abi.check(code, 'um_conv2d_entry_fwd')
        self.last_conv_stats = (st_t, parts)
        return t, d, ho, wo, (st_t, parts), (st_d, parts)

    def nhwc_planes_from(self, pieces, pad_to=32):
        rows = pieces[0].shape[0]
        c = sum(p.shape[1] for p in pieces)
        cp = (c + pad_to - 1) // pad_to * pad_to
        if cp != c:
            pieces = list(pieces) + [torch.zeros((rows, cp - c), dtype=torch.float32, device=pieces[0].device)]
        x = pieces[0].contiguous() if len(pieces) == 1 else torch.cat(list(pieces), 1)
        planes, _ = self.nhwc_norm(x, 1, rows, normalize=False, relu=False, want_planes=True)
        return planes, cp

    def conv_weight_padded(self, weight, cin_to):
        key, hit = self._cache_get(('padw', cin_to), (weight,))
        if hit is None:
            cout, cin, kh, kw = weight.shape
            wpad = torch.zeros((cout, cin_to, kh, kw), dtype=torch.float32, device=weight.device)
            wpad[:, :cin] = weight.detach().float()
            hit = self._cache_put(key, (weight,), wpad)
        return hit

    def planes_buffer(self, rows, ld):
        return torch.zeros(2 * (rows + 1) * ld * 2, dtype=torch.uint8, device='cuda')

    def cached_planes_buffer(self, tag, rows, ld, device):
        return self._workspace(('planes', tag), (rows, ld), 2 * (rows + 1) * ld * 2, torch.device(device), 1)

    def conv_weight_planes_from(self, weight):
        cout, cin, kh, kw = weight.shape
        w2 = weight.detach().float().permute(0, 2, 3, 1).reshape(cout, kh * kw * cin).contiguous()
        planes = torch.empty(self.lib.um_planes_bytes(cout, kh * kw * cin, 0), dtype=torch.uint8, device=w2.device)
        self._check_weight_range(w2, self.WSHIFT, 'convolution weight')
        _abi.check(self.lib.um_weight_planes(_ptr(w2), _ptr(planes), cout, kh * kw * cin, self.WSHIFT, 0, _stream()),
                   'um_weight_planes')
        return planes, cout, cin, kh, kw

    def conv_ex(self, src, geom, wb, ksize, stride, pad, act, out=None, outp=None):
        buf, a_ld, a_coff, cin = src
        b, h, w = geom
        (wp, cout, wcin, kh, kw), bias = wb
        if wcin != cin or (kh, kw) != tuple(ksize):
            raise ValueError(f'conv_ex: weight is {cout}x{wcin}x{kh}x{kw}, call wants cin={cin} k={ksize}')
        a_rows = buf.numel() // (4 * a_ld)
        ho, wo = (h + 2 * pad[0] - kh) // stride + 1, (w + 2 * pad[1] - kw) // stride + 1
        o_t, o_ld, o_coff = out if out is not None else (None, 0, 0)
        p_t, p_ld, p_coff = outp if outp is not None else (None, 0, 0)
        p_rows = p_t.numel() // (4 * p_ld) if p_t is not None else 0
        code = self._launch('conv', lambda: self.lib.um_conv2d_ex(
            _ptr(buf), a_ld, a_coff, a_rows, _ptr(wp), _ptr(bias) if bias is not None else None,
            _ptr(o_t) if o_t is not None else None, o_ld, o_coff, _ptr(p_t) if p_t is not None else None, p_ld, p_coff, p_rows,
            None, b, h, w, cin, cout, kh, kw, stride, pad[0], pad[1], act, self.WSHIFT, 0, _stream()),
            {'flops': 2.0 * b * ho * wo * cout * kh * kw * cin})
        _abi.check(code, 'um_conv2d_ex')

    def conv_gru(self, gate, src, geom, wb, ksize, pad, hidden, outp, z=None, z_out=None, addend=None, hidden_out=None):
        buf, a_ld, a_coff, cin = src
        b, h, w = geom
        (wp, cout, wcin, kh, kw), bias = wb
        c = hidden.shape[1]
        if wcin != cin or (kh, kw) != tuple(ksize) or cout != (2 * c if gate == 1 else c):
            raise ValueError('conv_gru: weight / hidden shapes do not match')
        p_t, p_ld, p_coff = outp
        zt = z if gate == 2 else None
# ... 39 lines not shown
        o_t, o_ld, o_coff = out if out is not None else (None, 0, 0)
        p_t, p_ld, p_coff = outp if outp is not None else (None, 0, 0)
        p_rows = p_t.numel() // (4 * p_ld) if p_t is not None else 0
        image = image.contiguous()
        code = self._launch('conv', lambda: self.lib.um_conv7_fwd(
            _ptr(image), c, 0, None, None, _ptr(scratch), _ptr(hit), _ptr(bias) if bias is not None else None,
            _ptr(o_t) if o_t is not None else None, o_ld, o_coff, _ptr(p_t) if p_t is not None else None, p_ld, p_coff, p_rows,
            None, b, h, w, cout, stride, act, self.WSHIFT, _stream()))
        _abi.check(code, 'um_conv7_fwd')

    def nhwc_gate(self, mode, src, dest, ld, coff, rows, channels, zr=None, hbuf=None):
        p_rows = dest.numel() // (4 * ld) if dest is not None else 0
        src_ld = src.shape[1] if src is not None else 0
        code = self._launch('instance_norm', lambda: self.lib.um_nhwc_gate(
            mode, _ptr(src) if src is not None else None, src_ld, _ptr(zr) if zr is not None else None,
            _ptr(hbuf) if hbuf is not None else None, _ptr(dest) if dest is not None else None, ld, coff, p_rows, rows, channels,
            _stream()))
        _abi.check(code, 'um_nhwc_gate')

    def local_corr_with_flow_planes(self, f0, f1, flow, h, w, radius, dest, ld):
        b, l, c = f0.shape
        _check_tokens('f0', f0, tokens=h * w)
        _check_tokens('f1', f1, b, l)
        flow = flow.contiguous()
        feat = self._k4_feat_planes(f0, f1, h, w, radius)
        if feat is not None:
            code = self._launch('local_corr_with_flow', lambda: self.lib.um_local_corr_with_flow_feat(
                _ptr(f0), _ptr(f1), _ptr(feat), _ptr(flow), None, _ptr(dest), ld, dest.numel() // (4 * ld), b, h, w, c, radius,
                self.k4_flags, None, _stream()))
            _abi.check(code, 'um_local_corr_with_flow_feat')
            return
        code = self._launch('local_corr_with_flow', lambda: self.lib.um_local_corr_with_flow_planes(
            _ptr(f0), _ptr(f1), _ptr(flow), _ptr(dest), ld, dest.numel() // (4 * ld), b, h, w, c, radius, _stream()))
        _abi.check(code, 'um_local_corr_with_flow_planes')

    k4_mfma = True
    k4_flags = 0

    def _k4_feat_planes(self, f0, f1, h, w, radius):
        if not self.k4_mfma or not self.lib.um_local_corr_with_flow_feat_supported(h, w, f0.shape[2], radius):
            return None
        key = (id(f0), f0._version, f0.data_ptr(), id(f1), f1._version, f1.data_ptr(), tuple(f0.shape))
        hit = getattr(self, '_k4_feat', None)
        if hit is not None and hit[0] == key and hit[1]() is f0 and hit[2]() is f1:
            return hit[3]
        b, l, c = f0.shape
        feat = torch.empty(self.lib.um_local_corr_feat_planes_bytes(b, h, w, c), dtype=torch.uint8, device=f0.device)
        _abi.check(self.lib.um_local_corr_feat_planes(_ptr(f0), _ptr(f1), _ptr(feat), b, h, w, c, _stream()),
                   'um_local_corr_feat_planes')
        self._k4_feat = (key, weakref.ref(f0), weakref.ref(f1), feat)
        return feat

    def stem_conv(self, image, weight, norm_mean_std=None, stats=True):
        if not (image.is_cuda and image.dtype == torch.float32 and image.dim() == 4 and image.shape[1] == 3
                and image.is_contiguous()):
            raise ValueError('stem_conv: expected a contiguous CUDA float32 [b, 3, h, w] image')
        if tuple(weight.shape[1:]) != (3, 7, 7):
            raise ValueError('stem_conv: expected a [cout, 3, 7, 7] weight')
        b, _, h, w = image.shape
        cout = weight.shape[0]
        key, hit = self._cache_get('stem', (weight,))
        if hit is None:
            wr = torch.zeros((cout, 7, 8, 4), dtype=torch.float32, device=weight.device)
            wr[:, :, :7, :3] = weight.detach().float().permute(0, 2, 3, 1)
            wr = wr.reshape(cout, 224).contiguous()
            wp = torch.empty(self.lib.um_planes_bytes(cout, 224, 0), dtype=torch.uint8, device=weight.device)
            self._check_weight_range(wr, self.WSHIFT, 'convolution weight')
            _abi.check(self.lib.um_weight_planes(_ptr(wr), _ptr(wp), cout, 224, self.WSHIFT, 0, _stream()), 'um_weight_planes')
            hit = self._cache_put(key, (weight,), wp)
        ho, wo = (h - 1) // 2 + 1, (w - 1) // 2 + 1
        scratch = torch.empty(self.lib.um_stem_planes_bytes(b, h, w), dtype=torch.uint8, device=image.device)
        out = torch.empty((b * ho * wo, cout), dtype=torch.float32, device=image.device)
        self.last_conv_stats = None
        if stats:
            parts = self.lib.um_conv_stats_parts(h, w, cout, 7, 7, 2, 3, 3)
            self.last_conv_stats = (torch.empty(self.lib.um_conv_stats_bytes(b, parts, cout) // 4, dtype=torch.float32,
                                                device=image.device), parts)
        st = self.last_conv_stats[0] if self.last_conv_stats is not None else None
        if norm_mean_std is not None:
            mean = (ctypes.c_float * 3)(*[float(v) for v in norm_mean_std[0]])
            std = (ctypes.c_float * 3)(*[float(v) for v in norm_mean_std[1]])
        else:
            mean = std = None
        code = self._launch('conv', lambda: self.lib.um_stem_conv_fwd(
            _ptr(image), int(norm_mean_std is not None), mean, std, _ptr(scratch), _ptr(hit), _ptr(out),
            _ptr(st) if st is not None else None, b, h, w, cout, self.WSHIFT, _stream()),
            {'flops': 2.0 * b * ho * wo * cout * 147})
        _abi.check(code, 'um_stem_conv_fwd')
        return out, ho, wo

    def nhwc_norm(self, x, b, pixels, normalize=True, relu=True, shortcut=None, want_planes=True, want_f32=False, eps=1e-5,
                  conv_stats=None, shortcut_planes=None, shortcut_stats=None):
        self._check_rows('x', x, x.shape[1])
        c = x.shape[1]
        if x.shape[0] != b * pixels:
            raise ValueError('nhwc_norm: x must have b * pixels rows')
        if shortcut is not None:
            self._check_rows('shortcut', shortcut, c)
        rows = b * pixels
        if shortcut_planes is not None and (shortcut is not None or shortcut_planes.numel() != self.lib.um_planes_bytes(rows + 1, c, self.CONV_MODE)):
            raise ValueError('nhwc_norm: shortcut_planes must be operand planes of [b * pixels + 1, c] (and exclude shortcut)')
        planes = (torch.empty(self.lib.um_planes_bytes(rows + 1, c, self.CONV_MODE), dtype=torch.uint8, device=x.device)
                  if want_planes else None)
        f32 = torch.empty_like(x) if want_f32 else None
        if shortcut_stats is not None:
            if shortcut is None or not normalize:
                raise ValueError('nhwc_norm: shortcut_stats go with an fp32 shortcut and normalize=True')
            ws = self._ws(self.lib.um_nhwc_norm_sc_workspace_bytes(b, pixels, c), x.device)
            code = self._launch('instance_norm', lambda: self.lib.um_nhwc_instance_norm_sc(
                _ptr(x), _ptr(shortcut), None, _ptr(planes) if planes is not None else None,
                _ptr(f32) if f32 is not None else None, b, pixels, c, float(eps), 1, int(bool(relu)),
                _ptr(conv_stats[0]) if conv_stats is not None else None, conv_stats[1] if conv_stats is not None else 0,
                _ptr(ws), ws.numel(), self.CONV_MODE, _stream(), _ptr(shortcut_stats[0]), shortcut_stats[1]))
            _abi.check(code, 'um_nhwc_instance_norm_sc')
            return planes, f32
        ws = self._ws(self.lib.um_nhwc_norm_workspace_bytes(b, pixels, c), x.device) if normalize else None
        code = self._launch('instance_norm', lambda: self.lib.um_nhwc_instance_norm(
            _ptr(x), _ptr(shortcut) if shortcut is not None else None,
            _ptr(shortcut_planes) if shortcut_planes is not None else None, _ptr(planes) if planes is not None else None,
            _ptr(f32) if f32 is not None else None, b, pixels, c, float(eps), int(bool(normalize)), int(bool(relu)),
            _ptr(conv_stats[0]) if conv_stats is not None else None, conv_stats[1] if conv_stats is not None else 0,
            _ptr(ws) if ws is not None else None, ws.numel() if ws is not None else 0, self.CONV_MODE, _stream()))
        _abi.check(code, 'um_nhwc_instance_norm')
        return planes, f32

    def nchw_to_nhwc(self, x, want_planes=True, want_f32=False):
        if not (x.is_cuda and x.dtype == torch.float32 and x.dim() == 4 and x.is_contiguous()):
            raise ValueError('nchw_to_nhwc: expected a contiguous CUDA float32 NCHW tensor')
        b, c, h, w = x.shape
        rows = b * h * w
        planes = (torch.empty(self.lib.um_planes_bytes(rows + 1, c, self.CONV_MODE), dtype=torch.uint8, device=x.device)
                  if want_planes else None)
        f32 = torch.empty((rows, c), dtype=torch.float32, device=x.device) if want_f32 else None
        code = self._launch('instance_norm', lambda: self.lib.um_nchw_to_nhwc(
            _ptr(x), _ptr(planes) if planes is not None else None, _ptr(f32) if f32 is not None else None, b, c, h * w,
            self.CONV_MODE, _stream()))
        _abi.check(code, 'um_nchw_to_nhwc')
        return planes, f32

    def global_corr_softmax_flow(self, f0, f1, h, w, bidir=False):
# ... 150 lines not shown
```

### unimatch_amd/streams.py

```python
import torch

from .dist import shard_bounds


def forward_parts(task, attn_type, num_scales, reg_refine, batch, height, width):
    if batch < 2:
        return 1
    size = batch * height * width / float(512 * 768)
    if reg_refine:
        need = 1.9 if task == 'flow' else 4.0
    elif attn_type and '1d' in attn_type:
        need = 6.0
    else:
        need = 2.8
    return 2 if size >= need else 1


_SIDE_STREAMS = {}


def _side_streams(dev, count):
    pool = _SIDE_STREAMS.setdefault(str(dev), [])
    while len(pool) < count:
        pool.append(torch.cuda.Stream(device=dev))
    return pool[:count]


class PartRunner:

    SEEN = 64

    def __init__(self):
        self._seen = set()
        self._backend = None

    @staticmethod
    def _backend_state(model):
        ops = getattr(model, '_ops', None)
        return (id(ops), getattr(ops, 'cache_generation', None))

    @staticmethod
    def _key(model, n, geometry, device, kw):
        version = sum(p._version for p in model.parameters())
        small = tuple(sorted((k, v if isinstance(v, (int, float, bool, str, type(None))) else
                              tuple(v) if isinstance(v, (list, tuple)) else tuple(v.shape)) for k, v in kw.items()))
        return (n, tuple(geometry), str(device), small, version)

    def run_parts(self, model, n, batch, bidir, geometry, device, kw, prepare, compute):
        cuda = device.type == 'cuda'

        def one(r, ins):
            if not cuda:
                return compute(r, ins)
            with model.ops.part_scope(r):
                return compute(r, ins)

        key = self._key(model, n, geometry, device, kw)
        concurrent = cuda and key in self._seen and self._backend is not None and self._backend == self._backend_state(model)
        if not concurrent:
            outs = [one(r, prepare(r)) for r in range(n)]
            if len(self._seen) >= self.SEEN:
                self._seen.clear()
            self._seen.add(key)
        else:
            cur = torch.cuda.current_stream(device)
            side = _side_streams(device, n - 1)
            ins = [prepare(r) for r in range(n)]
            for s in side:
                s.wait_stream(cur)
            outs = [None] * n
            try:
                for r in range(1, n):
                    with torch.cuda.stream(side[r - 1]):
                        outs[r] = one(r, ins[r])
                outs[0] = one(0, ins[0])
            finally:
                for s in side:
                    cur.wait_stream(s)
        self._backend = self._backend_state(model)
        counts = [shard_bounds(batch, r, n)[1] - shard_bounds(batch, r, n)[0] for r in range(n)]
        preds = []
        for i in range(len(outs[0])):
            pieces = [outs[r][i].reshape(bidir, counts[r], *outs[r][i].shape[1:]) for r in range(n)]
            preds.append(torch.cat(pieces, 1).reshape(bidir * batch, *outs[0][i].shape[1:]))
        if concurrent:
            if torch.cuda.is_current_stream_capturing():
                for r in range(1, n):
                    for t in outs[r]:
                        t.record_stream(cur)
            else:
                for s in side:
                    s.wait_stream(cur)
        return {'flow_preds': preds}


class ConcurrentUniMatch(torch.nn.Module):

    def __init__(self, model, parts=2):
        super().__init__()
        if parts < 1:
            raise ValueError('parts must be >= 1')
        self.model = model
        self.parts = parts

    @property
    def _backend(self):
        return self.model._runner._backend

    def forward(self, img0, img1, **kw):
        return self.model._forward_batch(img0, img1, self.parts, **kw)
```

Before: 970.3.

## Fuse image-pair stem conv, broadcast addend conv, concat planes, and direct output slices

Adds a stem conv entry that packs both images of a pair in one pack/conv launch, so the two images no longer need concatenating first. Adds a conv variant whose addend (such as a position embedding) is broadcast per image through an addend_period, a kernel that concatenates flow and tokens straight into fp16 planes, and lets each part write convex upsampling into a slice of a preallocated output so the final torch.cat is skipped. Each change removes a copy or an extra launch. In exchange it adds more API surface and templates the conv epilogue on a new ADDEND flag, which may change register use.

```diff
diff --git a/include/unimatch_hip.h b/include/unimatch_hip.h
--- a/include/unimatch_hip.h
+++ b/include/unimatch_hip.h
@@ -136,6 +136,9 @@
                           const float* addend, int addend_ld, float* hidden, const float* z, int z_ld, float* z_out, int z_out_ld,
                           void* out_planes, int outp_ld, int outp_coff, long outp_rows, int batch, int hi, int wi, int cin,
                           int channels, int kh, int kw, int pad_h, int pad_w, int wshift, int mode, void* stream);
+int um_conv2d_addend_fwd(const void* a_planes, const void* w_planes, const float* bias, const float* addend, int addend_ld,
+                         int addend_period, float* out, int batch, int hi, int wi, int cin, int cout, int kh, int kw, int stride,
+                         int pad_h, int pad_w, int wshift, int mode, void* stream);
 int um_conv_stats_parts(int hi, int wi, int cout, int kh, int kw, int stride, int pad_h, int pad_w);
 size_t um_conv_stats_bytes(int batch, int parts, int channels);
 
@@ -149,10 +152,17 @@
                      const void* w_planes, float* out, float* stats_out, int batch, int h, int w, int cout, int wshift,
                      void* stream);
 
+int um_stem_conv_pair_fwd(const float* image0, int batch0, const float* image1, int batch1, int normalize, const float* mean3,
+                          const float* std3, void* image_planes, const void* w_planes, float* out, float* stats_out, int h, int w,
+                          int cout, int wshift, void* stream);
+
 size_t um_nhwc_norm_workspace_bytes(int batch, int pixels, int channels);
 int um_nhwc_instance_norm(const float* x, const float* shortcut, const void* shortcut_planes, void* planes_out, float* f32_out,
                           int batch, int pixels, int channels, float eps, int normalize, int relu, const float* conv_stats,
                           int conv_stats_parts, void* workspace, size_t workspace_bytes, int mode, void* stream);
+
+int um_nhwc_concat_planes(const float* map, const float* tokens, void* planes_out, int batch, int pixels, int map_channels, int channels,
+                          int mode, void* stream);
 
 size_t um_nhwc_norm_sc_workspace_bytes(int batch, int pixels, int channels);
 int um_nhwc_instance_norm_sc(const float* x, const float* shortcut, const void* shortcut_planes, void* planes_out, float* f32_out,
diff --git a/unimatch_amd/_abi.py b/unimatch_amd/_abi.py
--- a/unimatch_amd/_abi.py
+++ b/unimatch_amd/_abi.py
@@ -39,6 +39,7 @@
                                 _c_size_t, _c_void_p]),
     'um_kv4_fwd': (_c_int, [_c_void_p, _c_void_p, _c_int, _c_int, _c_void_p, _c_int, _c_void_p]),
     'um_conv2d_fwd': (_c_int, [_c_void_p] * 5 + [_c_int] * 13 + [_c_void_p]),
+    'um_conv2d_addend_fwd': (_c_int, [_c_void_p] * 4 + [_c_int, _c_int, _c_void_p] + [_c_int] * 12 + [_c_void_p]),
     'um_conv2d_ex': (_c_int, [_c_void_p, _c_int, _c_int, ctypes.c_long, _c_void_p, _c_void_p, _c_void_p, _c_int, _c_int, _c_void_p,
                               _c_int, _c_int, ctypes.c_long, _c_void_p] + [_c_int] * 13 + [_c_void_p]),
     'um_nhwc_gate': (_c_int, [_c_int, _c_void_p, _c_int, _c_void_p, _c_void_p, _c_void_p, _c_int, _c_int, ctypes.c_long, ctypes.c_long,
@@ -63,6 +64,8 @@
     'um_conv7_fwd': (_c_int, [_c_void_p, _c_int, _c_int] + [_c_void_p] * 6 + [_c_int, _c_int, _c_void_p, _c_int, _c_int, ctypes.c_long,
                               _c_void_p] + [_c_int] * 7 + [_c_void_p]),
     'um_stem_conv_fwd': (_c_int, [_c_void_p, _c_int] + [_c_void_p] * 6 + [_c_int] * 5 + [_c_void_p]),
+    'um_stem_conv_pair_fwd': (_c_int, [_c_void_p, _c_int, _c_void_p, _c_int, _c_int] + [_c_void_p] * 6 + [_c_int] * 4 + [_c_void_p]),
+    'um_nhwc_concat_planes': (_c_int, [_c_void_p] * 3 + [_c_int] * 5 + [_c_void_p]),
     'um_nhwc_norm_workspace_bytes': (_c_size_t, [_c_int] * 3),
     'um_nhwc_instance_norm': (_c_int, [_c_void_p] * 5 + [_c_int] * 3 + [ctypes.c_float, _c_int, _c_int, _c_void_p, _c_int, _c_void_p,
                                        _c_size_t, _c_int, _c_void_p]),
diff --git a/unimatch_amd/csrc/conv.hip b/unimatch_amd/csrc/conv.hip
--- a/unimatch_amd/csrc/conv.hip
+++ b/unimatch_amd/csrc/conv.hip
@@ -27,6 +27,7 @@
     float* stats;
     const float* addend;
     int addend_ld;
+    int addend_period;
     int B, Hi, Wi, Cin, Ho, Wo, Cout;
     int KH, KW, stride, pad_h, pad_w;
     int M;
@@ -52,7 +53,7 @@
     static constexpr int value = V;
 };
 
-template <typename T, int NS, int NT, int NT0, int NTP, int WSTRIDE>
+template <typename T, int NS, int NT, int NT0, int NTP, int WSTRIDE, bool ADDEND>
 __device__ __forceinline__ void conv_epilogue_pass(const ConvArgs& a, f32x16 (&acc)[NT], unsigned char* lds, unsigned char* scratch,
                                                    int bt, int rloc0, int nvalid, int part0, bool dense_parts, int n0, int tid,
                                                    int wave, int lane, int half) {
@@ -70,7 +71,8 @@
     const int gate = a.gate;
     float* hbase = gate ? a.gate_h + rowbase * a.gate_c : nullptr;
     const float* zbase = gate == 2 ? a.gate_z + rowbase * a.gate_zld : nullptr;
-    const float* abase = a.addend ? a.addend + rowbase * a.addend_ld : nullptr;
+    const float* abase = ADDEND && a.addend ? a.addend + rowbase * a.addend_ld : nullptr;
+    const long aback = ADDEND && a.addend_period ? (long)bt * P * a.addend_ld : 0L;
     float* hobase = gate == 2 ? a.gate_hout + rowbase * a.gate_hout_ld : nullptr;
     f32x4 ad[NSIDE][BATCH], gz[NSIDE][BATCH], gh[NSIDE][BATCH];
     auto preload = [&](int b, int slot) {
@@ -81,7 +83,7 @@
             const int r = idx / CPR, c = idx - r * CPR;
             const int col = nb + 4 * c;
             if (r < nrows && col < a.Cout) {
-                if (abase) ad[slot][j] = *reinterpret_cast<const f32x4*>(abase + (unsigned)(r * a.addend_ld + col));
+                if (abase) ad[slot][j] = *reinterpret_cast<const f32x4*>(abase - aback + (unsigned)(r * a.addend_ld + col));
                 if (gate == 1 && col >= a.gate_c) gh[slot][j] = *reinterpret_cast<const f32x4*>(hbase + (unsigned)(r * a.gate_c + col - a.gate_c));
                 if (gate == 2) {
                     gz[slot][j] = *reinterpret_cast<const f32x4*>(zbase + (unsigned)(r * a.gate_zld + col));
@@ -117,7 +119,7 @@
         if (a.bias) to_lds(act_tag, IntC<1>{});
         else to_lds(act_tag, IntC<0>{});
     };
-    switch (a.addend ? 0 : a.act) {
+    switch (ADDEND && a.addend ? 0 : a.act) {
         case 0: to_lds_b(IntC<0>{}); break;
         case 1: to_lds_b(IntC<1>{}); break;
         case 2: to_lds_b(IntC<2>{}); break;
@@ -245,7 +247,7 @@
         }
     };
     auto store_rows_g = [&](auto gate_tag) {
-        if (a.addend) store_rows(gate_tag, IntC<1>{});
+        if (ADDEND && a.addend) store_rows(gate_tag, IntC<1>{});
         else store_rows(gate_tag, IntC<0>{});
     };
     if (a.gate == 0) store_rows_g(IntC<0>{});
@@ -253,15 +255,15 @@
     else store_rows_g(IntC<2>{});
 }
 
-template <typename T, int NS, int NT, int NTE = NT>
+template <typename T, int NS, int NT, int NTE = NT, bool ADDEND = true>
 __device__ __forceinline__ void conv_epilogue(const ConvArgs& a, f32x16 (&acc)[NT], unsigned char* lds, unsigned char* scratch,
                                               int bt, int rloc0, int nvalid, int part0, bool dense_parts, int n0, int tid, int wave,
                                               int lane, int half) {
     constexpr int NP = NTE < NT ? NTE : NT;
     constexpr int WSTRIDE = 32 * (32 * NP * 4);
-    conv_epilogue_pass<T, NS, NT, 0, NP, WSTRIDE>(a, acc, lds, scratch, bt, rloc0, nvalid, part0, dense_parts, n0, tid, wave, lane, half);
+    conv_epilogue_pass<T, NS, NT, 0, NP, WSTRIDE, ADDEND>(a, acc, lds, scratch, bt, rloc0, nvalid, part0, dense_parts, n0, tid, wave, lane, half);
     if constexpr (NTE < NT)
-        conv_epilogue_pass<T, NS, NT, NTE, NT - NTE, WSTRIDE>(a, acc, lds, scratch, bt, rloc0, nvalid, part0, dense_parts, n0, tid, wave,
+        conv_epilogue_pass<T, NS, NT, NTE, NT - NTE, WSTRIDE, ADDEND>(a, acc, lds, scratch, bt, rloc0, nvalid, part0, dense_parts, n0, tid, wave,
                                                               lane, half);
 }
 
@@ -529,7 +531,7 @@
 
     {
         const int rloc0 = pl0 + 32 * wave;
-        conv_epilogue<T, NS, NT>(a, acc, lds, lds + RING, bt, rloc0, min(32, max(0, P - rloc0)), bt * ((P + 127) / 128) + pl0 / 128, false,
+        conv_epilogue<T, NS, NT, NT, !ENTRY>(a, acc, lds, lds + RING, bt, rloc0, min(32, max(0, P - rloc0)), bt * ((P + 127) / 128) + pl0 / 128, false,
                                  n0, tid, wave, lane, half);
         if constexpr (ENTRY) {
             ConvArgs a2 = a;
@@ -537,7 +539,7 @@
             a2.out = e.out2;
             a2.stats = e.stats2;
             __syncthreads();
-            conv_epilogue<T, NS, NT>(a2, acc2, lds, lds + RING, bt, rloc0, min(32, max(0, P - rloc0)), bt * ((P + 127) / 128) + pl0 / 128,
+            conv_epilogue<T, NS, NT, NT, false>(a2, acc2, lds, lds + RING, bt, rloc0, min(32, max(0, P - rloc0)), bt * ((P + 127) / 128) + pl0 / 128,
                                      false, n0, tid, wave, lane, half);
         }
     }
@@ -1115,7 +1117,8 @@
                        float* stats_out, int batch, int hi, int wi, int cin, int cout, int kh, int kw, int stride,
                        int pad_h, int pad_w, int act, int wshift, int mode, void* stream_, int gate, float* gate_h,
                        const float* gate_z, int gate_zld, const float* addend = nullptr, int addend_ld = 0, float* gate_hout = nullptr,
-                       int gate_hout_ld = 0, const float* norm_x = nullptr, const float* norm_stats = nullptr, int norm_relu = 0) {
+                       int gate_hout_ld = 0, const float* norm_x = nullptr, const float* norm_stats = nullptr, int norm_relu = 0,
+                       int addend_period = 0) {
     const bool norm = norm_x != nullptr;
     if (gate_hout && (gate != 2 || gate_hout_ld < cout || gate_hout_ld % 4 != 0 || ((unsigned long)gate_hout & 15) != 0)) {
         um_set_error("um_conv2d: a separate new-state tensor goes with gate 2 only: 16-byte aligned fp32 [M][ld >= channels, ld %% 4 == 0]");
@@ -1193,6 +1196,7 @@
     a.stats = stats_out;
     a.addend = addend;
     a.addend_ld = addend_ld;
+    a.addend_period = addend_period;
     a.B = batch;
     a.Hi = hi;
     a.Wi = wi;
@@ -1288,6 +1292,19 @@
                         cin, cout, kh, kw, stride, pad_h, pad_w, relu ? 1 : 0, wshift, mode, stream_);
 }
 
+extern "C" int um_conv2d_addend_fwd(const void* a_planes, const void* w_planes, const float* bias, const float* addend, int addend_ld,
+                                    int addend_period, float* out, int batch, int hi, int wi, int cin, int cout, int kh, int kw, int stride,
+                                    int pad_h, int pad_w, int wshift, int mode, void* stream_) {
+    if (!addend || !out || (addend_period != 0 && addend_period != 1)) {
+        um_set_error("um_conv2d_addend_fwd: needs an addend, an fp32 output and addend_period 0 | 1");
+        return -1;
+    }
+    const long rows_in = (long)batch * hi * wi;
+    return conv2d_impl(a_planes, cin, 0, rows_in + 1, w_planes, bias, out, cout, 0, nullptr, 0, 0, 0, nullptr, batch, hi, wi, cin, cout, kh,
+                       kw, stride, pad_h, pad_w, 0, wshift, mode, stream_, 0, nullptr, nullptr, 0, addend, addend_ld, nullptr, 0, nullptr,
+                       nullptr, 0, addend_period);
+}
+
 extern "C" int um_conv2d_norm_fwd(const float* x, const float* norm_stats, int norm_relu, const void* w_planes, const float* bias, float* out,
                                   float* stats_out, int batch, int hi, int wi, int cin, int cout, int kh, int kw, int stride, int pad_h,
                                   int pad_w, int relu, int wshift, int mode, void* stream_) {
@@ -1367,7 +1384,7 @@
 }
 
 template <int CPP>
-__global__ __launch_bounds__(256) void pack7_kernel(const float* img, unsigned short* planes, long plane_stride, int B, int C,
+__global__ __launch_bounds__(256) void pack7_kernel(const float* img, const float* img1, int B0, unsigned short* planes, long plane_stride, int B, int C,
                                                     int H, int W, int Hp, int Wp, int normalize, float m0, float m1, float m2,
                                                     float s0, float s1, float s2) {
     const long idx = (long)blockIdx.x * 256 + threadIdx.x;
@@ -1382,10 +1399,12 @@
     for (int c = 0; c < CPP; ++c) v[c] = 0.f;
     if ((unsigned)y < (unsigned)H && (unsigned)x < (unsigned)W) {
         const float mean[3] = {m0, m1, m2}, sd[3] = {s0, s1, s2};
+        const float* src = b < B0 ? img : img1;
+        const int bl = b < B0 ? b : b - B0;
 #pragma unroll
         for (int c = 0; c < CPP; ++c) {
             if (c < C) {
-                float p = img[(((long)b * C + c) * H + y) * W + x];
+                float p = src[(((long)bl * C + c) * H + y) * W + x];
                 if (normalize && c < 3) p = (p / 255.0f - mean[c]) / sd[c];
                 v[c] = p;
             }
@@ -1409,13 +1428,13 @@
     return (size_t)(2 * ((long)batch * (h + 6) * conv7_wp(w) + 8) * cpp * 2);
 }
 
-extern "C" int um_conv7_fwd(const float* image, int channels, int normalize, const float* mean3, const float* std3,
-                            void* image_planes, const void* w_planes, const float* bias, float* out, int out_ld, int out_coff,
-                            void* out_planes, int outp_ld, int outp_coff, long outp_rows, float* stats_out, int batch, int h,
-                            int w, int cout, int stride, int act, int wshift, void* stream_) {
+static int conv7_impl(const float* image, const float* image1, int batch0, int channels, int normalize, const float* mean3, const float* std3,
+                      void* image_planes, const void* w_planes, const float* bias, float* out, int out_ld, int out_coff,
+                      void* out_planes, int outp_ld, int outp_coff, long outp_rows, float* stats_out, int batch, int h,
+                      int w, int cout, int stride, int act, int wshift, void* stream_) {
     hipStream_t stream = (hipStream_t)stream_;
     const int cpp = stride == 2 ? 4 : 8;
-    if (!image || !image_planes || !w_planes || (!out && !out_planes) || batch <= 0 || h < 7 || w < 7 || cout <= 0 || cout % 4 != 0 ||
+    if (!image || batch0 <= 0 || batch0 > batch || (batch0 < batch && !image1) || !image_planes || !w_planes || (!out && !out_planes) || batch <= 0 || h < 7 || w < 7 || cout <= 0 || cout % 4 != 0 ||
         wshift < 0 || wshift > 14 || (stride != 1 && stride != 2) || channels <= 0 || channels > (stride == 2 ? 3 : 8) ||
         (normalize && (!mean3 || !std3)) || act < 0 || act > 3) {
         um_set_error("um_conv7_fwd: bad argument (batch=%d channels=%d h=%d w=%d cout=%d stride=%d)", batch, channels, h, w, cout, stride);
@@ -1448,10 +1467,10 @@
         const float ss[3] = {normalize ? std3[0] : 1.f, normalize ? std3[1] : 1.f, normalize ? std3[2] : 1.f};
         const dim3 grid((unsigned)((rows + 255) / 256));
         if (cpp == 4)
-            hipLaunchKernelGGL((pack7_kernel<4>), grid, dim3(256), 0, stream, image, (unsigned short*)image_planes, plane_stride,
+            hipLaunchKernelGGL((pack7_kernel<4>), grid, dim3(256), 0, stream, image, image1, batch0, (unsigned short*)image_planes, plane_stride,
                                batch, channels, h, w, hp, wp, normalize, mm[0], mm[1], mm[2], ss[0], ss[1], ss[2]);
         else
-            hipLaunchKernelGGL((pack7_kernel<8>), grid, dim3(256), 0, stream, image, (unsigned short*)image_planes, plane_stride,
+            hipLaunchKernelGGL((pack7_kernel<8>), grid, dim3(256), 0, stream, image, image1, batch0, (unsigned short*)image_planes, plane_stride,
                                batch, channels, h, w, hp, wp, normalize, mm[0], mm[1], mm[2], ss[0], ss[1], ss[2]);
     }
     ConvArgs a;
@@ -1472,6 +1491,7 @@
     a.stats = stats_out;
     a.addend = nullptr;
     a.addend_ld = 0;
+    a.addend_period = 0;
     a.B = batch;
     a.Hi = hp;
     a.Wi = wp;
@@ -1505,6 +1525,14 @@
     return 0;
 }
 
+extern "C" int um_conv7_fwd(const float* image, int channels, int normalize, const float* mean3, const float* std3,
+                            void* image_planes, const void* w_planes, const float* bias, float* out, int out_ld, int out_coff,
+                            void* out_planes, int outp_ld, int outp_coff, long outp_rows, float* stats_out, int batch, int h,
+                            int w, int cout, int stride, int act, int wshift, void* stream_) {
+    return conv7_impl(image, nullptr, batch, channels, normalize, mean3, std3, image_planes, w_planes, bias, out, out_ld, out_coff, out_planes,
+                      outp_ld, outp_coff, outp_rows, stats_out, batch, h, w, cout, stride, act, wshift, stream_);
+}
+
 extern "C" size_t um_stem_planes_bytes(int batch, int h, int w) { return um_conv7_planes_bytes(batch, h, w, 2); }
 
 extern "C" int um_stem_conv_fwd(const float* image, int normalize, const float* mean3, const float* std3, void* image_planes,
@@ -1513,3 +1541,14 @@
     return um_conv7_fwd(image, 3, normalize, mean3, std3, image_planes, w_planes, nullptr, out, cout, 0, nullptr, 0, 0, 0, stats_out,
                         batch, h, w, cout, 2, 0, wshift, stream_);
 }
+
+extern "C" int um_stem_conv_pair_fwd(const float* image0, int batch0, const float* image1, int batch1, int normalize, const float* mean3,
+                                     const float* std3, void* image_planes, const void* w_planes, float* out, float* stats_out, int h, int w,
+                                     int cout, int wshift, void* stream_) {
+    if (!image0 || !image1 || batch0 <= 0 || batch1 <= 0) {
+        um_set_error("um_stem_conv_pair_fwd: two image tensors with a positive batch each (batch0=%d batch1=%d)", batch0, batch1);
+        return -1;
+    }
+    return conv7_impl(image0, image1, batch0, 3, normalize, mean3, std3, image_planes, w_planes, nullptr, out, cout, 0, nullptr, 0, 0, 0,
+                      stats_out, batch0 + batch1, h, w, cout, 2, 0, wshift, stream_);
+}
diff --git a/unimatch_amd/csrc/nhwc_ops.hip b/unimatch_amd/csrc/nhwc_ops.hip
--- a/unimatch_amd/csrc/nhwc_ops.hip
+++ b/unimatch_amd/csrc/nhwc_ops.hip
@@ -242,6 +242,43 @@
     }
 }
 
+template <typename T, int NS>
+__global__ __launch_bounds__(256) void nhwc_concat_planes_kernel(const float* map, const float* tokens, unsigned short* planes, long rows,
+                                                                 int P, int V, int C, int CP) {
+    __shared__ float tile[2048];
+    const int tpr = CP >> 3, R = 256 / tpr;
+    const long r0 = (long)blockIdx.x * R;
+    const long left = rows - r0;
+    const int nr = (int)(left < R ? (left > 0 ? left : 0) : R);
+    const f32x4* src = reinterpret_cast<const f32x4*>(tokens + r0 * C);
+    for (int i = threadIdx.x; i < nr * (C >> 2); i += 256) reinterpret_cast<f32x4*>(tile)[i] = src[i];
+    __syncthreads();
+    const int lr = threadIdx.x / tpr, j = threadIdx.x - lr * tpr;
+    const long row = r0 + lr;
+    if (lr >= R || row > rows) return;
+    const long plane_stride = (rows + 1) * CP;
+    unsigned short* dst = planes + row * CP + 8 * j;
+    if (row == rows) {
+        const u32x4 z = {0u, 0u, 0u, 0u};
+#pragma unroll
+        for (int pl = 0; pl < NS; ++pl) *reinterpret_cast<u32x4*>(dst + pl * plane_stride) = z;
+        return;
+    }
+    const long b = row / P, p = row - b * P;
+    float v[8], zf[8];
+#pragma unroll
+    for (int i = 0; i < 8; ++i) {
+        const int cc = 8 * j + i;
+        zf[i] = 0.f;
+        v[i] = cc < V ? map[(b * V + cc) * P + p] : cc < V + C ? tile[lr * C + cc - V] : 0.f;
+    }
+    const u32x4 z = {0u, 0u, 0u, 0u};
+    u32x4 h, l;
+    um_norm_value8<T, NS>(v, false, zf, zf, false, 0, zf, false, zf, zf, z, z, true, h, l);
+    *reinterpret_cast<u32x4*>(dst) = h;
+    if (NS == 2) *reinterpret_cast<u32x4*>(dst + plane_stride) = l;
+}
+
 __global__ __launch_bounds__(256) void nhwc_gate_kernel(int mode, const float* src, int src_ld, const float* zr, float* hbuf,
                                                         unsigned short* planes, long plane_stride, int ld, int coff, long rows,
                                                         int C) {
@@ -450,3 +487,32 @@
     }
     return 0;
 }
+
+extern "C" int um_nhwc_concat_planes(const float* map, const float* tokens, void* planes_out, int batch, int pixels, int map_channels,
+                                     int channels, int mode, void* stream_) {
+    hipStream_t stream = (hipStream_t)stream_;
+    if (!map || !tokens || !planes_out || batch <= 0 || pixels <= 0 || map_channels < 1 || map_channels > 4 || channels <= 0 ||
+        channels % 4 != 0 || channels > 256 || ((unsigned long)tokens & 15) != 0 || ((unsigned long)planes_out & 15) != 0 ||
+        (mode != 0 && mode != 1)) {
+        um_set_error("um_nhwc_concat_planes: bad argument (batch=%d pixels=%d map_channels=%d channels=%d: 1..4 map channels, token "
+                     "channels a multiple of 4, <= 256, 16-byte aligned tokens / planes)", batch, pixels, map_channels, channels);
+        return -1;
+    }
+    const long rows = (long)batch * pixels;
+    const int cp = (map_channels + channels + 31) / 32 * 32;
+    const int r = 256 / (cp / 8);
+    const dim3 grid((unsigned)((rows + 1 + r - 1) / r));
+    ScopedKernelTimer timer(UM_K_INSTANCE_NORM, stream);
+    if (mode == 0)
+        hipLaunchKernelGGL((nhwc_concat_planes_kernel<Fp16, 2>), grid, dim3(256), 0, stream, map, tokens, (unsigned short*)planes_out, rows,
+                           pixels, map_channels, channels, cp);
+    else
+        hipLaunchKernelGGL((nhwc_concat_planes_kernel<Bf16, 1>), grid, dim3(256), 0, stream, map, tokens, (unsigned short*)planes_out, rows,
+                           pixels, map_channels, channels, cp);
+    const hipError_t e = hipGetLastError();
+    if (e != hipSuccess) {
+        um_set_error("um_nhwc_concat_planes: launch failed: %s", hipGetErrorString(e));
+        return (int)e;
+    }
+    return 0;
+}
diff --git a/unimatch_amd/encoder.py b/unimatch_amd/encoder.py
--- a/unimatch_amd/encoder.py
+++ b/unimatch_amd/encoder.py
@@ -121,10 +121,16 @@
     def takes_raw_images(ops, x):
         return ops is not None and getattr(ops, 'fused_conv', False) and x.is_cuda
 
-    def forward(self, x, ops=None, input_norm=None):
-        if self.takes_raw_images(ops, x):
-            return self._forward_nhwc(x, ops, input_norm)
-        assert input_norm is None
+    def forward(self, x, ops=None, input_norm=None, out_addend=None):
+        if isinstance(x, (tuple, list)):
+            x = tuple(x)
+            pair = (len(x) == 2 and self.takes_raw_images(ops, x[0]) and getattr(ops, 'fused_glue', False)
+                    and x[0].shape[1:] == x[1].shape[1:] and x[0].dtype == x[1].dtype == torch.float32 and x[0].device == x[1].device)
+            if not pair:
+                x = x[0] if len(x) == 1 else torch.cat(x, 0)
+        if self.takes_raw_images(ops, x[0] if isinstance(x, tuple) else x):
+            return self._forward_nhwc(x, ops, input_norm, out_addend)
+        assert input_norm is None and out_addend is None
         if ops is not None and getattr(ops, 'fused_tail', False) and x.is_cuda:
             x = ops.instance_norm(self.conv1(x), relu=True)
             for layer in (self.layer1, self.layer2, self.layer3):
@@ -145,9 +151,14 @@
         s = blk.conv1.stride[0]
         return (h - 1) // s + 1, (w - 1) // s + 1, blk.conv1.out_channels
 
-    def _forward_nhwc(self, x, ops, input_norm=None):
-        b = x.shape[0]
-        y, h, w = ops.stem_conv(x.contiguous(), self.conv1.weight, input_norm, stats=True)
+    def _forward_nhwc(self, x, ops, input_norm=None, out_addend=None):
+        if isinstance(x, tuple):
+            b = x[0].shape[0] + x[1].shape[0]
+            x = tuple(t.contiguous() for t in x)
+        else:
+            b = x.shape[0]
+            x = x.contiguous()
+        y, h, w = ops.stem_conv(x, self.conv1.weight, input_norm, stats=True)
         c = y.shape[1]
         keep_f32 = self.shortcut_f32
         planes, f32 = ops.nhwc_norm(y, b, h * w, relu=True, want_planes=True, want_f32=keep_f32, conv_stats=ops.last_conv_stats)
@@ -158,7 +169,11 @@
             defer = nxt is not None and blk.downsample is None and nxt.entry_fusable(ops, *self._out_geometry(blk, act))
             act = blk.forward_nhwc(act, ops, want_f32=keep_f32 and nxt is not None and nxt.downsample is None, defer=defer)
         planes, _, b, h, w, c = act
-        out, _, _ = ops.conv2d_nhwc((planes, b, h, w, c), self.conv2.weight, self.conv2.bias, 1, (0, 0))
+        if out_addend is not None:
+            assert self.num_branch == 1, 'the trident branches read the position-free features'
+            out, _, _ = ops.conv2d_nhwc((planes, b, h, w, c), self.conv2.weight, self.conv2.bias, 1, (0, 0), image_addend=out_addend(h, w))
+        else:
+            out, _, _ = ops.conv2d_nhwc((planes, b, h, w, c), self.conv2.weight, self.conv2.bias, 1, (0, 0))
         if self.num_branch == 1:
             return [out.view(b, h, w, -1).permute(0, 3, 1, 2)]
         tp, _ = ops.nhwc_norm(out, b, h * w, normalize=False, relu=False, want_planes=True)
diff --git a/unimatch_amd/model.py b/unimatch_amd/model.py
--- a/unimatch_amd/model.py
+++ b/unimatch_amd/model.py
@@ -366,8 +366,15 @@
             b, v, h, w = flow2.shape
             rows = b * h * w
             feat = f0_map.permute(0, 2, 3, 1).reshape(rows, -1)
+            c1, c2 = self.upsampler[0], self.upsampler[2]
+            if getattr(ops, 'fused_glue', False) and v <= 4:
+                planes, cin = ops.nhwc_concat_planes(flow2.contiguous(), feat.contiguous())
+                hid = ops.cached_planes_buffer('upsampler_hidden', rows, c1.out_channels, flow2.device)
+                ops.conv_ex((planes, cin, 0, cin), (b, h, w), (ops.conv_weight_planes(ops.conv_weight_padded(c1.weight, cin)), c1.bias),
+                            (3, 3), 1, (1, 1), 1, outp=(hid, c1.out_channels, 0))
+                mask, _, _ = ops.conv2d_nhwc((hid, b, h, w, c1.out_channels), c2.weight, c2.bias, 1, (0, 0))
+                return mask, True
             planes, cin = ops.nhwc_planes_from([flow2.permute(0, 2, 3, 1).reshape(rows, v), feat])
-            c1, c2 = self.upsampler[0], self.upsampler[2]
             hid, _, _ = ops.conv2d_nhwc((planes, b, h, w, cin), ops.conv_weight_padded(c1.weight, cin), c1.bias, 1, (1, 1),
                                         relu=True)
             hp, hc = ops.nhwc_planes_from([hid])
@@ -375,10 +382,10 @@
             return mask, True
         return self.upsampler(torch.cat([flow2, f0_map], 1)), False
 
-    def _upsample(self, flow2, f0_map, is_depth=False):
+    def _upsample(self, flow2, f0_map, is_depth=False, out=None):
         mask, nhwc = self._upsample_mask(flow2, f0_map)
         if nhwc:
-            return self.ops.convex_upsample(flow2, mask, self.upsample_factor, is_depth, mask_nhwc=True)
+            return self.ops.convex_upsample(flow2, mask, self.upsample_factor, is_depth, mask_nhwc=True, out=out)
         return self._convex(flow2, mask, is_depth=is_depth)
 
     launch_parts = None
@@ -435,12 +442,15 @@
             pk = dict(kw, intrinsics=shard_batch(intrinsics, r, parts), pose=shard_batch(pose, r, parts))
             return shard_batch(img0, r, parts), shard_batch(img1, r, parts), pk
 
-        def compute(r, ins):
+        def compute(r, ins, out=None):
             a0, a1, pk = ins
-            return self._forward_one(a0, a1, **pk)['flow_preds']
+            return self._forward_one(a0, a1, pred_out=out, **pk)['flow_preds']
 
         bidir = 2 if (pred_bidir_flow or pred_bidir_depth) else 1
-        return self._runner.run_parts(self, parts, batch, bidir, img0.shape, img0.device, kw, prepare, compute)
+        out_shape = None
+        if task == 'flow' and bidir == 1 and img0.is_cuda and getattr(self.ops, 'fused_glue', False):
+            out_shape = (batch, 2) + tuple(img0.shape[-2:])
+        return self._runner.run_parts(self, parts, batch, bidir, img0.shape, img0.device, kw, prepare, compute, out_shape=out_shape)
 
     def _plan_parts(self, parts, task, attn_type, batch, height, width, is_cuda):
         if parts is None:
@@ -563,7 +573,7 @@
     def _forward_one(self, img0, img1, attn_type=None, attn_splits_list=None, corr_radius_list=None,
                      prop_radius_list=None, num_reg_refine=1, pred_bidir_flow=False, task='flow', intrinsics=None,
                      pose=None, min_depth=1. / 0.5, max_depth=1. / 10, num_depth_candidates=64,
-                     depth_from_argmax=False, pred_bidir_depth=False):
+                     depth_from_argmax=False, pred_bidir_depth=False, pred_out=None):
         if pred_bidir_flow:
             assert task == 'flow'
         if task == 'depth':
@@ -585,14 +595,17 @@
         if img1.device != dev:
             raise ValueError(f'img0 is on {dev} and img1 on {img1.device}')
         with guard, torch.no_grad():
-            feats = self._encode((img0, img1), task)
-            return self._match(feats, img0.shape[0], attn_type=attn_type, attn_splits_list=attn_splits_list,
+            with_pos = (self.num_scales == 1 and not self.reg_refine and self.debug_taps is None and getattr(ops, 'fused_glue', False)
+                        and self.backbone.takes_raw_images(ops, img0) and img0.shape == img1.shape)
+            pos = (lambda h, w: self._position(h, w, attn_splits_list[0], dev)) if with_pos else None
+            feats = self._encode((img0, img1), task, pos)
+            return self._match(feats, img0.shape[0], stream_has_pos=with_pos, pred_out=pred_out, attn_type=attn_type, attn_splits_list=attn_splits_list,
                                corr_radius_list=corr_radius_list, prop_radius_list=prop_radius_list, num_reg_refine=num_reg_refine,
                                pred_bidir_flow=pred_bidir_flow, task=task, intrinsics=intrinsics, pose=pose, min_depth=min_depth,
                                max_depth=max_depth, num_depth_candidates=num_depth_candidates, depth_from_argmax=depth_from_argmax,
                                pred_bidir_depth=pred_bidir_depth)
 
-    def _encode(self, images, task='flow'):
+    def _encode(self, images, task='flow', position=None):
         ops = self.ops
         input_norm = None
         if task == 'flow':
@@ -601,12 +614,17 @@
             else:
                 mean, std = self._constants(images[0].device)
                 images = tuple((im / 255. - mean) / std for im in images)
-        stack = images[0] if len(images) == 1 else torch.cat(images, 0)
+        pair = (len(images) == 2 and getattr(ops, 'fused_glue', False) and self.backbone.takes_raw_images(ops, images[0])
+                and images[0].shape == images[1].shape and images[0].dtype == images[1].dtype == torch.float32
+                and images[0].device == images[1].device)
+        stack = images[0] if len(images) == 1 else tuple(images) if pair else torch.cat(images, 0)
+        if position is not None:
+            return self.backbone(stack, ops, input_norm, out_addend=position)[::-1]
         return self.backbone(stack, ops, input_norm)[::-1]
 
     def _match(self, feats, nb, attn_type='', attn_splits_list=None, corr_radius_list=None, prop_radius_list=None, num_reg_refine=1,
                pred_bidir_flow=False, task='flow', intrinsics=None, pose=None, min_depth=1. / 0.5, max_depth=1. / 10,
-               num_depth_candidates=64, depth_from_argmax=False, pred_bidir_depth=False):
+               num_depth_candidates=64, depth_from_argmax=False, pred_bidir_depth=False, stream_has_pos=False, pred_out=None):
         ops = self.ops
         dev = feats[0].device
         flow, pred = None, None
@@ -642,8 +660,9 @@
             if self.debug_taps is not None:
                 self.debug_taps[f'backbone0_s{s}'], self.debug_taps[f'backbone1_s{s}'] = m0, m1
             if tok1 is ori1 and both is not None:
-                tok0, tok1 = self.transformer(ops, None, None, h, w, attn_type, splits, stream=both + pos)
+                tok0, tok1 = self.transformer(ops, None, None, h, w, attn_type, splits, stream=both if stream_has_pos else both + pos)
             else:
+                assert not stream_has_pos
                 tok0, tok1 = self.transformer(ops, ori0 + pos, tok1 + pos, h, w, attn_type, splits)
             if self.debug_taps is not None:
                 self.debug_taps[f'f0_s{s}'], self.debug_taps[f'f1_s{s}'] = _to_map(tok0, h, w), _to_map(tok1, h, w)
@@ -700,7 +719,7 @@
                     pad = torch.cat([flow, torch.zeros_like(flow)], 1)
                     pred = self._upsample(pad, f0_map, is_depth=True).clamp(min=min_depth, max=max_depth)[:, :1]
                 else:
-                    pred = self._upsample(flow, f0_map)
+                    pred = self._upsample(flow, f0_map, out=pred_out)
                 continue
             assert num_reg_refine > 0
             pose_r = pose
@@ -745,7 +764,8 @@
                         pred = self._upsample(pad, f0_map, is_depth=True).clamp(
                             min=min_depth, max=max_depth)[:, :1]
                     elif nhwc is not None:
-                        pred = ops.convex_upsample(flow, up_mask, self.upsample_factor, False, mask_nhwc=True)
+                        pred = ops.convex_upsample(flow, up_mask, self.upsample_factor, False, mask_nhwc=True,
+                                                   out=pred_out if task == 'flow' and not pred_bidir_flow else None)
                     else:
                         pred = self._convex(flow, up_mask)
         if task == 'stereo':
diff --git a/unimatch_amd/ops.py b/unimatch_amd/ops.py
--- a/unimatch_amd/ops.py
+++ b/unimatch_amd/ops.py
@@ -129,6 +129,7 @@
     fused_conv = True
     norm_on_load = True
     fused_entry = True
+    fused_glue = True
     CONV_MODE = 0
     WSHIFT = 10
 
@@ -388,13 +389,19 @@
         _abi.check(code, 'um_kv4_fwd')
         return out
 
-    def convex_upsample(self, flow, mask, factor, is_depth=False, mask_nhwc=False):
+    def convex_upsample(self, flow, mask, factor, is_depth=False, mask_nhwc=False, out=None):
         b, v, h, w = flow.shape
         want = (b * h * w, 9 * factor * factor) if mask_nhwc else (b, 9 * factor * factor, h, w)
         if not (flow.is_cuda and flow.dtype == torch.float32 and mask.dtype == torch.float32 and tuple(mask.shape) == want):
             raise ValueError(f'convex_upsample: bad shapes flow {tuple(flow.shape)} mask {tuple(mask.shape)}')
         flow, mask = flow.contiguous(), mask.contiguous()
-        up = torch.empty((b, v, factor * h, factor * w), dtype=torch.float32, device=flow.device)
+        up = out
+        if up is None:
+            up = torch.empty((b, v, factor * h, factor * w), dtype=torch.float32, device=flow.device)
+        elif not (tuple(up.shape) == (b, v, factor * h, factor * w) and up.dtype == torch.float32 and up.device == flow.device
+                  and up.is_contiguous()):
+            raise ValueError(f'convex_upsample: out must be a contiguous float32 [{b}, {v}, {factor * h}, {factor * w}] tensor on '
+                             f'{flow.device}, got {tuple(up.shape)} {up.dtype} {up.device}')
         code = self._launch('convex_upsample', lambda: self.lib.um_convex_upsample(
             _ptr(flow), _ptr(mask), _ptr(up), b, v, h, w, factor, int(bool(is_depth)), int(bool(mask_nhwc)), _stream()))
         _abi.check(code, 'um_convex_upsample')
@@ -594,7 +601,7 @@
                    'um_weight_planes')
         return self._cache_put(key, (weight,), (planes, cout, cin, kh, kw))
 
-    def conv2d_nhwc(self, act, weight, bias=None, stride=1, padding=(1, 1), relu=False, stats=False):
+    def conv2d_nhwc(self, act, weight, bias=None, stride=1, padding=(1, 1), relu=False, stats=False, image_addend=None):
         planes, b, h, w, cin = act
         wp, cout, wcin, kh, kw = self.conv_weight_planes(weight)
         if wcin != cin:
@@ -609,6 +616,18 @@
                                                 device=planes.device), parts)
         st = self.last_conv_stats[0] if self.last_conv_stats is not None else None
         meta = {'flops': 2.0 * b * ho * wo * cout * kh * kw * cin}
+        if image_addend is not None:
+            if relu or stats:
+                raise ValueError('conv2d_nhwc: image_addend excludes relu and stats')
+            if not (image_addend.is_cuda and image_addend.dtype == torch.float32 and image_addend.is_contiguous()
+                    and tuple(image_addend.shape) == (ho * wo, cout)):
+                raise ValueError(f'conv2d_nhwc: image_addend must be a contiguous CUDA float32 [{ho * wo}, {cout}] tensor, got '
+                                 f'{tuple(image_addend.shape)} {image_addend.dtype}')
+            code = self._launch('conv', lambda: self.lib.um_conv2d_addend_fwd(
+                _ptr(planes), _ptr(wp), _ptr(bias) if bias is not None else None, _ptr(image_addend), cout, 1, _ptr(out),
+                b, h, w, cin, cout, kh, kw, stride, ph, pw, self.WSHIFT, self.CONV_MODE, _stream()), meta)
+            _abi.check(code, 'um_conv2d_addend_fwd')
+            return out, ho, wo
         code = self._launch('conv', lambda: self.lib.um_conv2d_fwd(
             _ptr(planes), _ptr(wp), _ptr(bias) if bias is not None else None, _ptr(out), _ptr(st) if st is not None else None,
             b, h, w, cin, cout, kh, kw,
@@ -690,6 +709,23 @@
             pieces = list(pieces) + [torch.zeros((rows, cp - c), dtype=torch.float32, device=pieces[0].device)]
         x = pieces[0].contiguous() if len(pieces) == 1 else torch.cat(list(pieces), 1)
         planes, _ = self.nhwc_norm(x, 1, rows, normalize=False, relu=False, want_planes=True)
+        return planes, cp
+
+    def nhwc_concat_planes(self, flow, tokens, pad_to=32):
+        if pad_to != 32:
+            raise ValueError('nhwc_concat_planes: the kernel pads to 32 channels')
+        b, v, h, w = flow.shape
+        rows = b * h * w
+        self._check_rows('tokens', tokens, tokens.shape[1])
+        if not (flow.is_cuda and flow.dtype == torch.float32 and flow.is_contiguous() and tokens.shape[0] == rows):
+            raise ValueError(f'nhwc_concat_planes: expected a contiguous CUDA float32 flow [b, V, h, w] and tokens [b*h*w, C], got '
+                             f'{tuple(flow.shape)} {flow.dtype} and {tuple(tokens.shape)}')
+        c = tokens.shape[1]
+        cp = (v + c + 31) // 32 * 32
+        planes = torch.empty(self.lib.um_planes_bytes(rows + 1, cp, self.CONV_MODE), dtype=torch.uint8, device=flow.device)
+        code = self._launch('instance_norm', lambda: self.lib.um_nhwc_concat_planes(
+            _ptr(flow), _ptr(tokens), _ptr(planes), b, h * w, v, c, self.CONV_MODE, _stream()))
+        _abi.check(code, 'um_nhwc_concat_planes')
         return planes, cp
 
     def conv_weight_padded(self, weight, cin_to):
@@ -835,12 +871,23 @@
         return feat
 
     def stem_conv(self, image, weight, norm_mean_std=None, stats=True):
+        pair = None
+        if isinstance(image, (tuple, list)):
+            pair = tuple(image)
+            if len(pair) != 2 or pair[0].shape[1:] != pair[1].shape[1:] or pair[0].device != pair[1].device:
+                raise ValueError('stem_conv: a tuple holds two image tensors of one size on one device')
+            for im in pair[1:]:
+                if not (im.is_cuda and im.dtype == torch.float32 and im.dim() == 4 and im.shape[1] == 3 and im.is_contiguous()):
+                    raise ValueError('stem_conv: expected a contiguous CUDA float32 [b, 3, h, w] image')
+            image = pair[0]
         if not (image.is_cuda and image.dtype == torch.float32 and image.dim() == 4 and image.shape[1] == 3
                 and image.is_contiguous()):
             raise ValueError('stem_conv: expected a contiguous CUDA float32 [b, 3, h, w] image')
         if tuple(weight.shape[1:]) != (3, 7, 7):
             raise ValueError('stem_conv: expected a [cout, 3, 7, 7] weight')
         b, _, h, w = image.shape
+        if pair is not None:
+            b += pair[1].shape[0]
         cout = weight.shape[0]
         key, hit = self._cache_get('stem', (weight,))
         if hit is None:
@@ -865,10 +912,16 @@
             std = (ctypes.c_float * 3)(*[float(v) for v in norm_mean_std[1]])
         else:
             mean = std = None
+        meta = {'flops': 2.0 * b * ho * wo * cout * 147}
+        if pair is not None:
+            code = self._launch('conv', lambda: self.lib.um_stem_conv_pair_fwd(
+                _ptr(pair[0]), pair[0].shape[0], _ptr(pair[1]), pair[1].shape[0], int(norm_mean_std is not None), mean, std,
+                _ptr(scratch), _ptr(hit), _ptr(out), _ptr(st) if st is not None else None, h, w, cout, self.WSHIFT, _stream()), meta)
+            _abi.check(code, 'um_stem_conv_pair_fwd')
+            return out, ho, wo
         code = self._launch('conv', lambda: self.lib.um_stem_conv_fwd(
             _ptr(image), int(norm_mean_std is not None), mean, std, _ptr(scratch), _ptr(hit), _ptr(out),
-            _ptr(st) if st is not None else None, b, h, w, cout, self.WSHIFT, _stream()),
-            {'flops': 2.0 * b * ho * wo * cout * 147})
+            _ptr(st) if st is not None else None, b, h, w, cout, self.WSHIFT, _stream()), meta)
         _abi.check(code, 'um_stem_conv_fwd')
         return out, ho, wo
 
diff --git a/unimatch_amd/streams.py b/unimatch_amd/streams.py
--- a/unimatch_amd/streams.py
+++ b/unimatch_amd/streams.py
@@ -46,14 +46,18 @@
                               tuple(v) if isinstance(v, (list, tuple)) else tuple(v.shape)) for k, v in kw.items()))
         return (n, tuple(geometry), str(device), small, version)
 
-    def run_parts(self, model, n, batch, bidir, geometry, device, kw, prepare, compute):
+    def run_parts(self, model, n, batch, bidir, geometry, device, kw, prepare, compute, out_shape=None):
         cuda = device.type == 'cuda'
+        full = slices = None
+        if out_shape is not None and bidir == 1 and cuda:
+            full = torch.empty(tuple(out_shape), dtype=torch.float32, device=device)
+            slices = [full[slice(*shard_bounds(batch, r, n))] for r in range(n)]
 
         def one(r, ins):
             if not cuda:
                 return compute(r, ins)
             with model.ops.part_scope(r):
-                return compute(r, ins)
+                return compute(r, ins) if slices is None else compute(r, ins, out=slices[r])
 
         key = self._key(model, n, geometry, device, kw)
         concurrent = cuda and key in self._seen and self._backend is not None and self._backend == self._backend_state(model)
@@ -78,6 +82,8 @@
                 for s in side:
                     cur.wait_stream(s)
         self._backend = self._backend_state(model)
+        if slices is not None and all(len(outs[r]) == 1 and outs[r][0] is slices[r] for r in range(n)):
+            return {'flow_preds': [full]}
         counts = [shard_bounds(batch, r, n)[1] - shard_bounds(batch, r, n)[0] for r in range(n)]
         preds = []
         for i in range(len(outs[0])):
```

Result: faster. 987.7, median of 6 (+1.8%).
